# muhd-umer/ltr-lowrank-sdp

Measured on AMD Instinct MI355X. Metric: ALM iters/sec, MaxCut G67 (torus 100x100 +-1, n=m=10000), fixed default rank, higher is better.
Workload: dtype f64; 1 GPU; MaxCut torus 100x100 (G67 structure); n=10000, m=10000, rank=19, pattern_slots=30000, constraint_nnz=10000, flags=--fixedRank 19 --reoptLevel 0, phase-1 exit disabled, budget = steps, parallelism=none (1 GPU)

## Files before the change

include/lrsdp.h:

```cpp
#ifndef LRSDP_H
#define LRSDP_H
#define LRSDP_ABI_VERSION 2
#ifdef __cplusplus
extern "C" {
#endif

typedef struct lrs_ctx lrs_ctx;
typedef struct lrs_loopback lrs_loopback;

typedef struct {
    double initRho, rhoMax, rhoCellingALM, rhoCellingADMM;
    int maxALMIter, maxADMMIter;
    double timesLogRank;
    int fixedRank, initRank, rhoFreq;
    double rhoFactor, ALMRhoFactor, rankUpdateFactor, phase1Tol, phase2Tol, timeSecLimit, heuristicFactor;
    int lbfgsListLength;
    double endTauTol, endALMSubTol;
    int l2Rescaling, reoptLevel, dyrankLevel, highAccMode, oracleRankNaive;
    int disableOracle;
    double nearStallFactor;
    const int *rankSchedule;
    int rankScheduleLen;
    int verbose;
    long almInnerBudget;
    int skipADMM;
} lrs_params;

typedef struct {
    long alm_inner, alm_outer, admm_iter, cg_iter;
    double alm_pobj, alm_dobj, alm_pinf, alm_gap, alm_rho;
    double pobj, dobj, pinf, pinf_inf, gap, rho;
    double solve_time, alm_time, admm_time, read_time;
    int status;
    int retcode;
    int final_rank, oracle_rank;
    int traj1_len, traj2_len;
    double rho_max;
    double dinf, dinf_inf, dinf_2;
    int dinf_converged;
    int dinf_iters;
    long dinf_steps;
    double dinf_time;
    double obj_scale;
} lrs_result;

enum { LRS_R = 0, LRS_D = 1, LRS_G = 2, LRS_U = 3, LRS_V = 4, LRS_S0 = 5, LRS_Y0 = 6, LRS_S1 = 7, LRS_Y1 = 8 };
enum { LRS_LAMBDA = 0, LRS_CVS = 1, LRS_Q1 = 2, LRS_Q2 = 3, LRS_B = 4 };

void lrs_params_default(lrs_params *p);
const char *lrs_last_error(void);
const char *lrs_version(void);
int lrs_abi_version(void);

int lrs_ctx_create(int device, lrs_ctx **out);
void lrs_ctx_destroy(lrs_ctx *ctx);

int lrs_load_sdpa(lrs_ctx *ctx, const char *path, double *read_seconds);
int lrs_problem_info(lrs_ctx *ctx, int *m, int *ncones, int *dims, long *nslots, long *nnz_constraints);

int lrs_determine_rank(lrs_ctx *ctx, const lrs_params *p, int *ranks_out);
int lrs_set_rank(lrs_ctx *ctx, const int *ranks);
int lrs_get_rank(lrs_ctx *ctx, int *ranks);

int lrs_factor_set(lrs_ctx *ctx, int which, const double *colmajor);
int lrs_factor_get(lrs_ctx *ctx, int which, double *colmajor);
int lrs_vec_set(lrs_ctx *ctx, int which, const double *v);
int lrs_vec_get(lrs_ctx *ctx, int which, double *v);

int lrs_op_q12(lrs_ctx *ctx, double *q1, double *p1, double *q2, double *p2);
int lrs_op_constr_rr(lrs_ctx *ctx, double *cvs, double *pinf, double *pobj);
int lrs_op_grad(lrs_ctx *ctx, double rho, double *lag_norm_sq);
int lrs_op_line_search(lrs_ctx *ctx, double rho, double *tau, int *root_num);
int lrs_op_lbfgs(lrs_ctx *ctx, int node_num, double beta_new, double beta_old);
int lrs_op_admm_constr(lrs_ctx *ctx);
int lrs_op_admm_half(lrs_ctx *ctx, int cone, int side, double rho, double cg_tol, int cg_maxit, int *cg_iters,
                     double *rhs);
int lrs_op_dual_update(lrs_ctx *ctx, double rho);
int lrs_op_alm_update(lrs_ctx *ctx, double rho, double tau, double *lag_norm_sq, double *beta);
int lrs_op_adjoint(lrs_ctx *ctx, const double *y, int which, double *out, double scale, int with_C);
int lrs_op_auv(lrs_ctx *ctx, int u, int v, double *out_m, double *cobj);
int lrs_op_dimacs(lrs_ctx *ctx, int admm, double *out5);
int lrs_op_gram(lrs_ctx *ctx, int cone, int which, double *gram);
int lrs_op_dual_infeasibility(lrs_ctx *ctx, double *l1, double *lam_min);

int lrs_solve(lrs_ctx *ctx, const lrs_params *p, lrs_result *res);
int lrs_trajectory(lrs_ctx *ctx, int phase, int *curr_rank, int *oracle_rank, int cap);
int lrs_write_json(lrs_ctx *ctx, const char *path, const char *problem_id, const char *file_path,
                   const lrs_result *res, const lrs_params *p);

int lrs_alm_throughput(lrs_ctx *ctx, const lrs_params *p, long warmup, long steps, double *seconds,
                       long *done, double *sddmm_avg_ms, double *iter_avg_ms);

typedef long (*lrs_budget_hook)(void *user, long inner_done);
int lrs_set_budget_hook(lrs_ctx *ctx, lrs_budget_hook hook, void *user);
int lrs_alm_last_step(lrs_ctx *ctx, double *out4, int *newest_pair);
int lrs_sync(lrs_ctx *ctx);

int lrs_set_log_path(lrs_ctx *ctx, const char *path);

int lrs_set_kernel_path(lrs_ctx *ctx, int path);
int lrs_get_kernel_path(lrs_ctx *ctx, int *used);

int lrs_time_auut(lrs_ctx *ctx, int reps, double *avg_ms);
int lrs_auut_bytes(lrs_ctx *ctx, double *bytes);

int lrs_time_gram(lrs_ctx *ctx, int cone, int reps, double *avg_ms, double *gram_ms);

int lrs_mfma_f64_peak(lrs_ctx *ctx, double *tflops);
int lrs_mfma_f64_probe(lrs_ctx *ctx, int waves_per_simd, int chains, double *tflops, double *mhz,
                       double *cycles_per_mfma);

int lrs_time_dense(lrs_ctx *ctx, int cone, int reps, double *avg_ms);

int lrs_dense_a_info(lrs_ctx *ctx, int cone, int *n_dense, int *on_dense_path, long *stack_bytes);
int lrs_time_dense_a(lrs_ctx *ctx, int cone, int reps, double *avg_ms);
int lrs_dense_a_plan(const char *path, int cone, int *n_dense, int *on_dense_path, int *cons, int cap);

int lrs_rank1_info(lrs_ctx *ctx, int cone, int *n_rank1, int *on_factor_path, long *factor_bytes);
int lrs_rank1_plan(const char *path, int cone, int *n_rank1, int *on_factor_path, int *cons, double *sigma, int cap);
int lrs_time_rank1(lrs_ctx *ctx, int cone, int reps, double *avg_ms, double *bytes);
int lrs_load_coo_rank1(lrs_ctx *ctx, int m, int nblk, const int *dims, const double *b, long nnz, const int *con,
                       const int *blk, const int *row, const int *col, const double *val, int nterm, const int *tcon,
                       const int *tblk, const double *tsigma, const double *tvec);

int lrs_profile_stages(lrs_ctx *ctx, const lrs_params *p, long steps, double *stage_ms, long *done);

int lrs_load_coo(lrs_ctx *ctx, int m, int nblk, const int *dims, const double *b, long nnz, const int *con,
                 const int *blk, const int *row, const int *col, const double *val);

int lrs_tile_info(lrs_ctx *ctx, int *auv, int *slot);
int lrs_tile_used(lrs_ctx *ctx, int *used);

int lrs_stage_bytes(lrs_ctx *ctx, double *bytes);

int lrs_time_stages(lrs_ctx *ctx, int reps, double *stage_ms);

int lrs_debug_phase_times(lrs_ctx *ctx, unsigned long long *out, unsigned long long *blk);

int lrs_comm_unique_id(char *id_out);
int lrs_shard_rccl(lrs_ctx *ctx, int world, int rank, const char *id);
int lrs_loopback_create(int world, lrs_loopback **out);
void lrs_loopback_destroy(lrs_loopback *g);
int lrs_shard_loopback(lrs_ctx *ctx, lrs_loopback *g, int rank);
int lrs_shard_info(lrs_ctx *ctx, int *world, int *rank, int *row0, int *nown, int *nhalo);
int lrs_shard_comm_ranks(lrs_ctx *ctx, int *count);
int lrs_shard_comm_record(lrs_ctx *ctx, int on);
int lrs_xwg_fallbacks(lrs_ctx *ctx, int *count);
int lrs_shard_comm_log(lrs_ctx *ctx, long *out, long cap, long *n);
int lrs_shard_plan(const char *path, int world, int rank, long *counts, int *bounds, int *local_gid,
                   int *send_ptr, int *send_gid, int *shared_gid, int *con_gid, int *primary);

#ifdef __cplusplus
}
#endif
#endif
```

ltr-lowrank-sdp_amd/csrc/lrs_device.h:

```cpp
#pragma once
#include <hip/hip_runtime.h>

#include <cstdint>
#include <string>
#include <vector>

namespace lrs {

constexpr int kBlock = 256;
constexpr int kMaxPartialBlocks = 4096;
constexpr int kMaxPartialVals = 16;

enum CtrlIdx {
    C_ACTIVE = 0,
    C_EXIT,
    C_INNER,
    C_LOCAL,
    C_CLEAR,
    C_HEAD,
    C_GCUR,
    C_PENDING,
    C_RCVAL,
    C_LAG,
    C_PINF1,
    C_PINFINF,
    C_BETA0, C_BETA1,
    C_YY0, C_YY1,
    C_NODENUM,
    C_CG, C_CS0, C_CY0, C_CS1, C_CY1,
    C_DG,
    C_LASTTAU,
    C_DSG, C_DYG, C_DSOG, C_DYOG, C_DSOY, C_DYOY,
    C_ACT2,
    C_EXIT2,
    C_RRDONE,
    C_RCUR,
    C_NCTRL = 40
};
enum ExitReason {
    EXIT_NONE = 0,
    EXIT_CONVERGED = 1,
    EXIT_PHASE1 = 2,
    EXIT_LOCAL800 = 3,
    EXIT_TINYTAU = 4,
    EXIT_NUMERR = 5,
    EXIT_BUDGET = 6,
    EXIT_XWG = 7
};
enum ParIdx {
    P_RHO = 0, P_RCTOL, P_ENDSUB, P_ENDTAU, P_PH1TOL, P_BN1, P_BNINF, P_CNINF,
    P_HIGHACC, P_BUDGET, P_L, P_GAP, P_NPAR = 16
};
enum LsIdx { LS_TAU = 0, LS_ROOTNUM, LS_FLAG, LS_N = 4 };
constexpr int kMaxCones = 256;
constexpr int kFinN = 416;
enum TmpFinIdx {
    TF_SD = 0, TF_GATHER = 2 * kMaxCones, TF_RESID, TF_DOT, TF_DOTC, TF_SPMM = TF_DOTC + kMaxCones,
    TF_N = TF_SPMM + kMaxCones
};
constexpr int kMaxShards = 64;
constexpr int kLongRow = 32;

struct Layout {
    int G = 1, E = 1, ld = 1;
};
Layout choose_layout(int r);

struct DevCone {
    int n = 0, r = 0, ld = 0, G = 0, E = 0;
    bool lp = false;
    int *lp_slot = nullptr;
    double *lp_nrm2 = nullptr;
    int row0 = 0, nown = 0;
    long foff = 0;
    int slot_off = 0, P = 0;
    int *adj_ptr = nullptr, *adj_low = nullptr, *adj_col = nullptr, *adj_slot = nullptr;
    long adj_nnz = 0;
    bool auv_diag = false;
    int maxdeg = 0, maxlow = 0;
    std::vector<int> dra_h, drb_h;
    std::vector<int> dra_n, drb_n;
    int *dra = nullptr, *drb = nullptr;
    long gl_need = 0;
    int dense_c = 0;
    double *Cd = nullptr;
    double c_alpha = 0.0;
    int kd = 0;
    double *dA = nullptr;
    int *dA_con = nullptr;
    std::vector<int> dA_con_h;
    const double *dSd = nullptr;
    int rp = 0, rldp = 0;
    double *rV = nullptr, *r_sigma = nullptr;
    int *r_con = nullptr;
    const double *r1w = nullptr;
    double *r1T = nullptr, *r1part = nullptr;
    int *colseg = nullptr;
    int auv_items = 0;
    long auv_ebase = 0;
    int *auv_item = nullptr;
    unsigned *auv_pq = nullptr;
    int *auv_pos = nullptr;
    double *auv_val = nullptr;
    int sa_items = 0;
    int sa_n = 0;
    int *sa_item = nullptr;
    int sa_nsub = 0;
    int *sa_sub = nullptr;
    int sa_ngrp = 0;
    int *sa_grp = nullptr;
    unsigned *sa_pq = nullptr;
    int *sa_slot = nullptr;
    int sb_blocks = 0;
    int *sb_blk = nullptr, *sb_tp = nullptr, *sb_rp = nullptr, *sb_ent = nullptr;
    double *sa_S = nullptr;
    int sb_I0 = 0;
    int sx_n = 0;
    int *sx_slot = nullptr;
    int cg_ok = 0, cg_ncs = 0, cg_ncl = 0, cg_ns = 0, cg_nce = 0, cg_nsc = 0, cg_nadj = 0, cg_cconst = 0, cg_cslot = 0;
    int *cg_cadj_ptr = nullptr, *cg_cadj = nullptr, *cg_cl_con = nullptr, *cg_cl_ptr = nullptr, *cg_ce = nullptr;
    int *cg_sp = nullptr, *cg_sj = nullptr, *cg_cc_ptr = nullptr, *cg_cc = nullptr;
    double *cg_ce_w = nullptr, *cg_sa = nullptr;
    int cobj_n = 0;
    int *cobj_slot = nullptr;
};
constexpr int kScMaxN = 256;
constexpr int kMaxRankLd = 512;
constexpr int kAuvT = 128;
constexpr int kAuvC = 32;
constexpr int kAuvThreads = 512;
constexpr int kAuvNpt = 8;
constexpr int kAuvItem = kAuvThreads * kAuvNpt;
constexpr int kTileSub = 1024;
constexpr int kTileGrp = 2;
constexpr int kAuvMinN = 2048;
constexpr int kAuvMinPerTile = 768;
constexpr int kCgSplitSlabs = 8;
constexpr int kNX = 8;
constexpr int kTileMinDeg = 32;
constexpr int kDenseRow = 64;
constexpr int kSliceMinB = 28;
constexpr int kMaxDenseRows = 32;

struct ShardHooks {
    void *self = nullptr;
    int (*halo)(void *self, double *D, hipStream_t st) = nullptr;
    int (*allreduce)(void *self, double *buf, int n, hipStream_t st) = nullptr;
};

struct DevProblem {
    const ShardHooks *shard = nullptr;
    int no_lat = 0;
    int *slot_g = nullptr;
    mutable int last_path = -1;
    mutable int last_tiles = 0;
    int m = 0, K = 0;
    int lp_cone = -1;
    long NRpad = 0;
    int Ptot = 0;
    long Z = 0;
    double *b = nullptr;
    double *Cw = nullptr, *Craw = nullptr;
    int *con_ptr = nullptr, *con_slot = nullptr;
    double *con_w = nullptr;
    int *slot_ptr = nullptr, *slot_con = nullptr;
    double *slot_a = nullptr;
    int mg = 0;
    int glob_maxlen = 0;
    int *glob = nullptr;
    int *loc_ptr = nullptr, *loc_con = nullptr;
    double *loc_w = nullptr;
    int *slot_rc = nullptr;
    double *slot1 = nullptr;
    double *loc1 = nullptr;
    int *con1_pq = nullptr;
    int *long_rows = nullptr;
    std::vector<int> long_ptr_h;
    double *con1_w = nullptr;
    int nsh = 0;
    int *sh_idx = nullptr;
    double *cmask = nullptr;
    double *bprim = nullptr;
    double *g3 = nullptr;
    double *gpack = nullptr;
    double *spack = nullptr;
    std::vector<DevCone> cones;
    int ndense = 0;
    int ndensea = 0;
    bool tiles = false;
    double *gp = nullptr;
    double *cgk = nullptr;
    double dense_scale = 1.0;
    DevCone merged;
    bool has_merged = false;
    bool cone_sep = false;
};

struct DevWork {
    double *R = nullptr, *D = nullptr, *G[2] = {nullptr, nullptr};
    double *R2 = nullptr;
    double *CR = nullptr, *CD = nullptr;
    double *CGK = nullptr;
    double *dT = nullptr, *dSd = nullptr, *dpart = nullptr;
    double *rTx = nullptr, *rTz = nullptr, *rTy = nullptr, *rpart = nullptr;
    double *GP = nullptr;
    double *ls[2] = {nullptr, nullptr}, *ly[2] = {nullptr, nullptr};
    double *U = nullptr, *V = nullptr, *X = nullptr;
    double *cg_r = nullptr, *cg_p = nullptr, *cg_Q = nullptr, *cg_b = nullptr, *M2 = nullptr;
    double *uvt0 = nullptr, *uvt1 = nullptr, *uvt2 = nullptr, *S = nullptr;
    double *uvp = nullptr;
    double *lam = nullptr, *cvs = nullptr, *q1 = nullptr, *q2 = nullptr, *M1 = nullptr, *wtmp = nullptr;
    double *cvc = nullptr;
    double *lpw = nullptr;
    double *part = nullptr;
    double *partB = nullptr;
    double *partC = nullptr;
    double *ctrl = nullptr;
    double *lsres = nullptr;
    double *par = nullptr;
    double *gram = nullptr;
    double *rec = nullptr;
    double *cgc = nullptr;
    double *tot = nullptr;
    double *gl = nullptr;
    long gl_len = 0;
};


int launch_sddmm(const DevProblem &P, int cone, int mode, const double *X, const double *Y,
                 double *out0, double *out1, double *part, int pblk_off, int *nblk_used,
                 hipStream_t st);
int launch_gather(const DevProblem &P, const double *uvt, double scale, double *out,
                  const double *b_for_vio, double *vio_part, hipStream_t st, int *nblk_used);
int launch_auv_con(const DevProblem &P, int cone, int mode, const double *X, const double *Y, double scale,
                   int accumulate, double *out, const double *b_for_vio, double *vio_part, hipStream_t st,
                   const double *guard = nullptr, double *sum_upd = nullptr);
int launch_cobj(const DevProblem &P, int cone, int mode, const double *X, const double *Y, double *part,
                hipStream_t st);
// ... 103 lines not shown
```

ltr-lowrank-sdp_amd/csrc/lrs_kernels.hip:

```cpp
#include <hip/hip_runtime.h>
#include <utility>

#include <cmath>
#include <cstdio>
#include <cstring>
#include <cstdlib>
#include <algorithm>

#include "lrs_device.h"

namespace lrs {

static thread_local char g_err[512] = "";

#ifdef LRS_PHASE_TIMING
__device__ unsigned long long g_phase[4][16];
__device__ unsigned long long g_phase_tmp[4][16];
#define LRS_TS(k, p)                                                                  \
    do {                                                                              \
        if (blockIdx.x == 0 && threadIdx.x == 0) g_phase_tmp[k][p] = wall_clock64();  \
    } while (0)
#define LRS_TS_END(k, p)                                                              \
    do {                                                                              \
        if (blockIdx.x == 0 && threadIdx.x == 0) {                                    \
            g_phase_tmp[k][p] = wall_clock64();                                       \
            for (int q_ = 0; q_ <= (p); ++q_) g_phase[k][q_] = g_phase_tmp[k][q_];    \
        }                                                                             \
    } while (0)
__device__ unsigned long long g_blk[4][1024][2];
#define LRS_BLK_BEGIN() const unsigned long long t_begin_ = wall_clock64()
#define LRS_BLK_END(k)                                                                 \
    do {                                                                               \
        if (threadIdx.x == 0 && blockIdx.x < 1024) {                                   \
            g_blk[k][blockIdx.x][0] = t_begin_;                                        \
            g_blk[k][blockIdx.x][1] = wall_clock64();                                  \
        }                                                                              \
    } while (0)
#else
#define LRS_TS(k, p) do { } while (0)
#define LRS_TS_END(k, p) do { } while (0)
#define LRS_BLK_BEGIN() do { } while (0)
#define LRS_BLK_END(k) do { } while (0)
#endif
int read_phase_times(unsigned long long *out, unsigned long long *blk) {
#ifdef LRS_PHASE_TIMING
    if (hipMemcpyFromSymbol(out, HIP_SYMBOL(g_phase), sizeof(g_phase)) != hipSuccess) return -1;
    if (blk && hipMemcpyFromSymbol(blk, HIP_SYMBOL(g_blk), sizeof(g_blk)) != hipSuccess) return -1;
    return 64;
#else
    (void)out;
    (void)blk;
    return 0;
#endif
}
const char *last_device_error() { return g_err; }

#define LRS_CHECK_LAUNCH()                                                               \
    do {                                                                                 \
        hipError_t e_ = hipGetLastError();                                               \
        if (e_ != hipSuccess) {                                                          \
            snprintf(g_err, sizeof(g_err), "%s:%d %s", __FILE__, __LINE__, hipGetErrorString(e_)); \
            return (int)e_;                                                              \
        }                                                                                \
    } while (0)

Layout choose_layout(int r) {
    if (const char *e = getenv("LRS_LAYOUT")) {
        int g = 0, el = 0;
        if (sscanf(e, "%dx%d", &g, &el) == 2 && (g == 8 || g == 16 || g == 32 || g == 64) && el >= 1 && el <= 4 &&
            g * el >= r) {
            Layout f;
            f.G = g; f.E = el; f.ld = g * el;
            return f;
        }
    }
    static const int Gs[4] = {8, 16, 32, 64};
    static const int Es[4] = {2, 1, 4, 3};
    Layout best;
    best.ld = 1 << 30;
    for (int ei = 0; ei < 4; ++ei)
        for (int gi = 0; gi < 4; ++gi) {
            int ld = Gs[gi] * Es[ei];
            if (ld >= r && ld < best.ld) { best.G = Gs[gi]; best.E = Es[ei]; best.ld = ld; }
        }
    if (best.ld > 512 && r <= 512) { best.G = 64; best.E = 8; best.ld = 512; }
    return best;
}

template <int CTRL>
__device__ __forceinline__ double dpp_mov(double v) {
    const long long b = __double_as_longlong(v);
    const int lo = __builtin_amdgcn_mov_dpp((int)b, CTRL, 0xF, 0xF, false);
    const int hi = __builtin_amdgcn_mov_dpp((int)(b >> 32), CTRL, 0xF, 0xF, false);
    return __longlong_as_double(((long long)hi << 32) | (unsigned int)lo);
}

__device__ __forceinline__ double opaque(double x) {
    asm volatile("" : "+v"(x));
    return x;
}

template <int G>
__device__ __forceinline__ double group_sum(double v) {
    v += dpp_mov<0xB1>(v);
    v += dpp_mov<0x4E>(v);
    if constexpr (G >= 8) v += dpp_mov<0x141>(v);
    if constexpr (G >= 16) v += dpp_mov<0x140>(v);
    if constexpr (G >= 32) v += __shfl_xor(v, 16, 64);
    if constexpr (G >= 64) v += __shfl_xor(v, 32, 64);
    return v;
}

template <int G>
__device__ __forceinline__ double group_sum4(const double (&d)[4], int o) {
    static_assert(G == 4 || G == 16, "group of 4 or 16 lanes");
    if constexpr (G == 4) {
        const bool h1 = (o & 2) != 0, h0 = (o & 1) != 0;
        double a0 = h1 ? d[2] : d[0], a1 = h1 ? d[3] : d[1];
        a0 += dpp_mov<0x4E>(h1 ? d[0] : d[2]);
        a1 += dpp_mov<0x4E>(h1 ? d[1] : d[3]);
        return (h0 ? a1 : a0) + dpp_mov<0xB1>(h0 ? a0 : a1);
    } else {
        const bool h3 = (o & 8) != 0, h2 = (o & 4) != 0;
        double a0 = h3 ? d[2] : d[0], a1 = h3 ? d[3] : d[1];
        a0 += dpp_mov<0x140>(h3 ? d[0] : d[2]);
        a1 += dpp_mov<0x140>(h3 ? d[1] : d[3]);
        double v = (h2 ? a1 : a0) + dpp_mov<0x141>(h2 ? a0 : a1);
        v += dpp_mov<0x4E>(v);
        v += dpp_mov<0xB1>(v);
        return v;
    }
}

__device__ __forceinline__ double read_lane(double v, int l) {
    const long long b = __double_as_longlong(v);
    const int lo = __builtin_amdgcn_readlane((int)b, l);
    const int hi = __builtin_amdgcn_readlane((int)(b >> 32), l);
    return __longlong_as_double(((long long)hi << 32) | (unsigned int)lo);
}

template <int G>
__device__ __forceinline__ int bcast_i(int v, int u) {
    if constexpr (G == 64) return __builtin_amdgcn_readlane(v, u);
    else return __shfl(v, (int)(threadIdx.x & 63 & ~(G - 1)) + u, 64);
}
template <int G>
__device__ __forceinline__ double bcast_d(double v, int u) {
    if constexpr (G == 64) return read_lane(v, u);
    else return __shfl(v, (int)(threadIdx.x & 63 & ~(G - 1)) + u, 64);
}

__device__ __forceinline__ double wave_sum(double v) {
    v = group_sum<16>(v);
    return (read_lane(v, 0) + read_lane(v, 16)) + (read_lane(v, 32) + read_lane(v, 48));
}

template <int E>
__device__ __forceinline__ void ld_row(const double *__restrict__ p, double (&v)[E]) {
    if constexpr (E == 2) {
        double2 t = *reinterpret_cast<const double2 *>(p);
        v[0] = t.x; v[1] = t.y;
    } else if constexpr (E == 4) {
        double2 t0 = reinterpret_cast<const double2 *>(p)[0];
        double2 t1 = reinterpret_cast<const double2 *>(p)[1];
        v[0] = t0.x; v[1] = t0.y; v[2] = t1.x; v[3] = t1.y;
    } else {
#pragma unroll
        for (int e = 0; e < E; ++e) v[e] = p[e];
    }
}

template <int E>
__device__ __forceinline__ void st_row(double *__restrict__ p, const double (&v)[E]) {
    if constexpr (E == 2) {
        *reinterpret_cast<double2 *>(p) = make_double2(v[0], v[1]);
    } else if constexpr (E == 4) {
        reinterpret_cast<double2 *>(p)[0] = make_double2(v[0], v[1]);
        reinterpret_cast<double2 *>(p)[1] = make_double2(v[2], v[3]);
    } else {
#pragma unroll
        for (int e = 0; e < E; ++e) p[e] = v[e];
    }
}

template <int NV, int NT = kBlock>
__device__ __forceinline__ void block_reduce(double (&acc)[NV], double (&s)[NV]) {
    __shared__ double sh[NV][NT / 64];
    const int wid = threadIdx.x >> 6, lane = threadIdx.x & 63;
#pragma unroll
    for (int v = 0; v < NV; ++v) {
        double t = wave_sum(acc[v]);
        if (lane == 0) sh[v][wid] = t;
    }
    __syncthreads();
    if (threadIdx.x == 0) {
#pragma unroll
        for (int v = 0; v < NV; ++v) {
            double t = 0.0;
#pragma unroll
            for (int w = 0; w < NT / 64; ++w) t += sh[v][w];
            s[v] = t;
        }
    }
    __syncthreads();
}

template <int NV>
__device__ void partials_finalize(double (&acc)[NV], double *__restrict__ part, unsigned *ticket,
                                  double *__restrict__ fin, int *inc = nullptr) {
    double s[NV];
    block_reduce<NV>(acc, s);
    __shared__ unsigned is_last;
    if (threadIdx.x == 0) {
#pragma unroll
        for (int v = 0; v < NV; ++v) part[v * kMaxPartialBlocks + blockIdx.x] = s[v];
        asm volatile("s_waitcnt vmcnt(0)" ::: "memory");
        __builtin_amdgcn_fence(__ATOMIC_RELEASE, "agent");
        asm volatile("s_waitcnt vmcnt(0)" ::: "memory");
        unsigned t = __hip_atomic_fetch_add(ticket, 1u, __ATOMIC_RELAXED, __HIP_MEMORY_SCOPE_AGENT);
        is_last = (t == gridDim.x - 1) ? 1u : 0u;
    }
    __syncthreads();
    if (!is_last) return;
    if (threadIdx.x == 0) {
        __builtin_amdgcn_fence(__ATOMIC_ACQUIRE, "agent");
        asm volatile("s_waitcnt vmcnt(0)" ::: "memory");
    }
    __syncthreads();
    double a2[NV];
#pragma unroll
    for (int v = 0; v < NV; ++v) {
        double t = 0.0;
        for (int b = threadIdx.x; b < (int)gridDim.x; b += kBlock) t += part[v * kMaxPartialBlocks + b];
        a2[v] = t;
    }
    double s2[NV];
    block_reduce<NV>(a2, s2);
    if (threadIdx.x == 0) {
#pragma unroll
        for (int v = 0; v < NV; ++v) fin[v] = s2[v];
        if (inc) *inc = *inc + 1;
        __hip_atomic_store(ticket, 0u, __ATOMIC_RELAXED, __HIP_MEMORY_SCOPE_AGENT);
    }
}

static inline int grid_rows(long rows, int G) {
    long threads = rows * G;
    long b = (threads + kBlock - 1) / kBlock;
    if (b < 1) b = 1;
    if (b > kMaxPartialBlocks) b = kMaxPartialBlocks;
    return (int)b;
}
static inline int grid_elems(long n, int per_thread) {
    long b = (n / per_thread + kBlock - 1) / kBlock;
    if (b < 1) b = 1;
    if (b > kMaxPartialBlocks) b = kMaxPartialBlocks;
    return (int)b;
}

enum TicketId { T_SDDMM = 0, T_GATHER, T_SPMM, T_DOT, T_GRAD, T_RR, T_Q, T_NT = 16 };

// ... 816 lines not shown
    }
    if (delta < 0) {
        const double sqA = sqrt(A);
        const double T = (A * b - 1.5 * a * B) / (A * sqA);
        const double th = acos(T);
        const double cs = cos(th / 3), sn = sqrt(3.0) * sin(th / 3);
        res[0] = (-b - 2 * sqA * cs) / 3 / a;
        res[1] = (-b + sqA * (cs + sn)) / 3 / a;
        res[2] = (-b + sqA * (cs - sn)) / 3 / a;
        return 3;
    }
    return 0;
}

__device__ __forceinline__ int dev_cubic_wave(double a, double b, double c, double d, double *res) {
    const double A = b * b - 3 * a * c, B = b * c - 9 * a * d, C = c * c - 3 * b * d;
    const double delta = B * B - 4 * A * C;
    res[0] = res[1] = res[2] = 0.0;
    if (A == 0 && B == 0) { res[0] = fmax(res[0], -c / b); return 1; }
    if (delta > 0) {
        const double sq = sqrt(delta);
        const double Y1 = A * b + 1.5 * a * (-B + sq);
        const double Y2 = A * b + 1.5 * a * (-B - sq);
        const double y = (threadIdx.x & 1) ? Y2 : Y1;
        const double ay = y > 0 ? y : -y;
        double r = pow(ay, 1.0 / 3);
        r = y > 0 ? r : -r;
        const double Y13 = read_lane(r, 0), Y23 = read_lane(r, 1);
        res[0] = fmax(res[0], (-b - Y13 - Y23) / 3 / a);
        return 1;
    }
    if (delta == 0 && A != 0 && B != 0) {
        const double Kk = B / A;
        res[0] = -b / a + Kk; res[1] = -Kk / 2;
        return 2;
    }
    if (delta < 0) {
        const double sqA = sqrt(A);
        const double T = (A * b - 1.5 * a * B) / (A * sqA);
        const double th = acos(T);
        double sn, cs;
        sincos(th / 3, &sn, &cs);
        sn *= sqrt(3.0);
        res[0] = (-b - 2 * sqA * cs) / 3 / a;
        res[1] = (-b + sqA * (cs + sn)) / 3 / a;
        res[2] = (-b + sqA * (cs - sn)) / 3 / a;
        return 3;
    }
    return 0;
}

__device__ __forceinline__ double quartic(double a, double b, double c, double d, double x) {
    const double x2 = x * x;
    return a * (x2 * x2) + b * (x2 * x) + c * x2 + d * x;
}

__device__ void line_search_v(const double *__restrict__ par, double p1, double p2, const double *dots, double *ls);
__device__ void line_search(const double *__restrict__ par, int K, const double *__restrict__ fin, double *ls) {
    double p1 = 0.0, p2 = 0.0;
    for (int k = 0; k < K; ++k) { p1 += fin[FIN_SD + 2 * k]; p2 += fin[FIN_SD + 2 * k + 1]; }
    double dots[5];
    for (int q = 0; q < 5; ++q) dots[q] = fin[FIN_Q + q];
    line_search_v(par, p1, p2, dots, ls);
}
template <int NV, int NT = kBlock>
__device__ __forceinline__ void write_partials(double (&acc)[NV], double *__restrict__ part, int slot) {
    __shared__ double sh[NV][NT / 64];
    const int wid = threadIdx.x >> 6, lane = threadIdx.x & 63;
#pragma unroll
    for (int v = 0; v < NV; ++v) {
        const double t = wave_sum(acc[v]);
        if (lane == 0) sh[v][wid] = t;
    }
    __syncthreads();
    if (threadIdx.x < NV) {
        const int v = threadIdx.x;
        double t = 0.0;
#pragma unroll
        for (int w = 0; w < NT / 64; ++w) t += sh[v][w];
        part[v * kMaxPartialBlocks + slot] = t;
    }
}

template <int NV>
__device__ __forceinline__ void write_partials_nw(double (&acc)[NV], double *__restrict__ part, int slot, int nw) {
    __shared__ double sh[NV][8];
    const int wid = threadIdx.x >> 6, lane = threadIdx.x & 63;
#pragma unroll
    for (int v = 0; v < NV; ++v) {
        const double t = wave_sum(acc[v]);
        if (lane == 0) sh[v][wid] = t;
    }
    __syncthreads();
    if (threadIdx.x < NV) {
        const int v = threadIdx.x;
        double t = 0.0;
#pragma unroll
        for (int w = 0; w < 8; ++w)
            if (w < nw) t += sh[v][w];
        part[v * kMaxPartialBlocks + slot] = t;
    }
}

template <int NV, int NT = kBlock>
__device__ __forceinline__ void write_partials_range(double (&acc)[NV], double *__restrict__ part, int slot, int v0,
                                                     int v1) {
    double s[NV];
    block_reduce<NV, NT>(acc, s);
    if (threadIdx.x == 0) {
#pragma unroll
        for (int v = 0; v < NV; ++v)
            if (v >= v0 && v < v1) part[v * kMaxPartialBlocks + slot] = s[v];
    }
}

template <int NV, int NT = kBlock>
__device__ __forceinline__ void reduce_partials(const double *__restrict__ part, int nblk, double *out,
                                                int pstr = kMaxPartialBlocks) {
    double a[NV];
#pragma unroll
    for (int v = 0; v < NV; ++v) a[v] = 0.0;
    for (int b = threadIdx.x; b < nblk; b += NT) {
#pragma unroll
        for (int v = 0; v < NV; ++v) a[v] += part[v * pstr + b];
    }
    double s[NV];
    block_reduce<NV, NT>(a, s);
    if (threadIdx.x == 0) {
#pragma unroll
        for (int v = 0; v < NV; ++v) out[v] = s[v];
    }
    __syncthreads();
}

template <bool WAVE, typename PB>
__device__ __forceinline__ void line_search_t(const PB &par, double p1, double p2, const double *dots, double *ls) {
    p1 *= 2.0;
    const double rho = par[P_RHO];
    const double a = rho * dots[0] / 2;
    const double b = rho * dots[1];
    const double c = p2 - rho * dots[2] + rho * dots[3] / 2;
    const double d = p1 - rho * dots[4];
    double roots[3];
    const int rn = WAVE ? dev_cubic_wave(4 * a, 3 * b, 2 * c, d, roots) : dev_cubic(4 * a, 3 * b, 2 * c, d, roots);
    double tau = 0.0;
    const double f0 = 0.0, f1 = quartic(a, b, c, d, 1.0);
    double fr1 = 1e30, fr2 = 1e30, fr3 = 1e30;
    if (rn >= 1 && roots[0] > 1e-20 && roots[0] <= 1.0) fr1 = quartic(a, b, c, d, roots[0]);
    if (rn >= 2 && roots[1] > 1e-20 && roots[1] <= 1.0) fr2 = quartic(a, b, c, d, roots[1]);
    if (rn == 3 && roots[2] > 1e-20 && roots[2] <= 1.0) fr3 = quartic(a, b, c, d, roots[2]);
    const double mn = fmin(fmin(fmin(fmin(f0, f1), fr1), fr2), fr3);
    if (fabs(mn - f0) < 1e-10) tau = 0.0;
    if (fabs(mn - f1) < 1e-10) tau = 1.0;
    if (fabs(mn - fr1) < 1e-10) tau = roots[0];
    if (fabs(mn - fr2) < 1e-10) tau = roots[1];
    if (fabs(mn - fr3) < 1e-10) tau = roots[2];
    if (!WAVE || (threadIdx.x & 63) == 0) {
        ls[LS_TAU] = tau;
        ls[LS_ROOTNUM] = rn;
        ls[LS_FLAG] = rn == 0 ? 1.0 : (fabs(tau) < par[P_ENDTAU] ? 2.0 : 0.0);
    }
}
__device__ void line_search_v(const double *__restrict__ par, double p1, double p2, const double *dots, double *ls) {
    line_search_t<false>(par, p1, p2, dots, ls);
}

template <typename CB, typename PB>
__device__ __forceinline__ void ctrl_step(CB &&c, const PB &par, double lsflag, double lstau, int fold,
                                          const double *d, bool ph1) {
    const int L = (int)par[P_L];
    const double cninf = par[P_CNINF], rctol = par[P_RCTOL], endsub = par[P_ENDSUB], budget = par[P_BUDGET];
    c[C_ACTIVE] = c[C_ACT2];
    c[C_EXIT] = c[C_EXIT2];
    c[C_RRDONE] = 0.0;
    if (c[C_ACTIVE] != 0.0 && c[C_PENDING] == 1.0) {
        if (lsflag == 1.0) {
            c[C_ACTIVE] = 0.0; c[C_EXIT] = EXIT_NUMERR;
            c[C_PENDING] = 0.0;
        } else if (lsflag == 2.0) {
            c[C_INNER] += 1; c[C_LOCAL] += 1; c[C_CLEAR] += 1;
            c[C_ACTIVE] = 0.0; c[C_EXIT] = EXIT_TINYTAU;
            c[C_PENDING] = 0.0;
        } else if (fold) {
            const int h = (int)c[C_HEAD];
// ... 998 lines not shown
            }
            st_row<E>(CRb + foff + oi, cr);
        }
        double sv2[E], yv[E];
#pragma unroll
        for (int e = 0; e < E; ++e) g[e] *= 2.0;
#pragma unroll
        for (int e = 0; e < E; ++e) { sv2[e] = tau * w.di[e]; yv[e] = g[e] - go[e]; }
        st_row<E>(Gnew + oi, g);
        st_row<E>(sh + oi, sv2);
        st_row<E>(yh + oi, yv);
#pragma unroll
        for (int e = 0; e < E; ++e) {
            acc[0] += g[e] * g[e];
            acc[1] += yv[e] * sv2[e];
            acc[2] += yv[e] * yv[e];
            acc[3] += sv2[e] * g[e];
            acc[4] += yv[e] * g[e];
        }
        if (two) {
#pragma unroll
            for (int e = 0; e < E; ++e) {
                acc[5] += sov[e] * g[e];
                acc[6] += yov[e] * g[e];
                acc[7] += sov[e] * yv[e];
                acc[8] += yov[e] * yv[e];
            }
        }
    }
    LRS_TS(2, 3);
    write_partials<10, kRowBlock>(acc, partC, pblk_off + blockIdx.x);
    LRS_TS_END(2, 4);
    LRS_BLK_END(2);
}

__device__ __forceinline__ int lat_row_block(int b, int nrb) {
#ifndef LRS_NO_LAT_XCD
    if (b >= nrb || nrb < 16) return b;
    const int x = b & 7, q8 = nrb >> 3, rem = nrb & 7;
    const int start = x * q8 + min(x, rem);
    return start + (b >> 3);
#else
    (void)nrb;
    return b;
#endif
}
constexpr int kLatNT = 512;
constexpr int kLatRowWaves = kLatNT / 64 - 1;
constexpr int kLatRows = kLatRowWaves * 64;
constexpr int kLatMaxPartials = 256;
constexpr int kSliceA = 2;
constexpr int kSliceB = 4;

constexpr int kLatQ = kLatMaxPartials / 64;
template <int NV>
__device__ __forceinline__ void load_partials(const double *__restrict__ part, int nblk, double (&x)[kLatQ][NV]) {
    const int lane = threadIdx.x & 63;
#pragma unroll
    for (int q = 0; q < kLatQ; ++q) {
        const int bc = min(lane + 64 * q, nblk - 1);
#pragma unroll
        for (int v = 0; v < NV; ++v) x[q][v] = part[v * kMaxPartialBlocks + bc];
    }
}
template <int NV>
__device__ __forceinline__ void sum_partials(const double (&x)[kLatQ][NV], int nblk, double (&out)[NV]) {
    const int lane = threadIdx.x & 63;
#pragma unroll
    for (int v = 0; v < NV; ++v) {
        double a = 0.0;
#pragma unroll
        for (int q = 0; q < kLatQ; ++q) a += (lane + 64 * q < nblk) ? x[q][v] : 0.0;
        out[v] = wave_sum(a);
    }
}
template <int NV>
__device__ __forceinline__ void wave_reduce_partials(const double *__restrict__ part, int nblk, double (&out)[NV]) {
    double x[kLatQ][NV];
    load_partials<NV>(part, nblk, x);
    __builtin_amdgcn_sched_barrier(0);
    sum_partials<NV>(x, nblk, out);
}

template <int G, int E, int NO>
__global__ void __launch_bounds__(kLatNT) k_lat_a(
    int n, int ld, long foff, const int *__restrict__ adj_ptr, const int *__restrict__ adj_low,
    const int *__restrict__ adj_col, const int *__restrict__ adj_slot, const double *__restrict__ Cw,
    const double *__restrict__ Rb0, const double *__restrict__ Rb1, double *__restrict__ Dall,
    const double *__restrict__ G0, const double *__restrict__ G1, const double *__restrict__ s0a,
    const double *__restrict__ y0a, const double *__restrict__ s1a, const double *__restrict__ y1a,
    double *__restrict__ uRD, double *__restrict__ uDD, const int *__restrict__ loc_ptr,
    const int *__restrict__ loc_con, const double *__restrict__ loc_w, const double2 *__restrict__ loc1,
    const double *__restrict__ b, double *__restrict__ cvs, const double *__restrict__ lam,
    double *__restrict__ rec, int do_glob, int mg, const int *__restrict__ glob, int m, int K,
    const int *__restrict__ con_ptr, const int *__restrict__ con_slot, const double *__restrict__ con_w,
    const double *__restrict__ uRR, const double *__restrict__ par, const double *__restrict__ ctrl_prev,
    double *__restrict__ ctrl_cur, const double *__restrict__ ls_prev, const double *__restrict__ partC, int nblkC,
    double *__restrict__ partA, int pblk_off, int gwide, int nrb, int lrw, int nda, const int *__restrict__ dra) {
    __shared__ double c[C_NCTRL];
    __shared__ double pl[P_NPAR];
    LRS_TS(0, 0);
    LRS_BLK_BEGIN();
    const int nwv = lrw + 1, rpb = lrw * 64 / G;
    const bool ctrl_wave = __builtin_amdgcn_readfirstlane((int)(threadIdx.x >> 6)) == nwv - 1;
    const int lane = threadIdx.x & (G - 1);
    const bool slice = (int)blockIdx.x >= nrb;
    int i = lat_row_block((int)blockIdx.x, nrb) * rpb + (int)threadIdx.x / G, sq = 0;
    if (slice) {
        const int per = rpb * kSliceA;
        int q = (int)blockIdx.x - nrb, L = 0;
        for (; L < nda - 1; ++L) {
            const int r = dra[L], ns = (adj_low[r] - adj_ptr[r] + per - 1) / per;
            if (q < ns) break;
            q -= ns;
        }
        i = dra[L];
        sq = q * per + ((int)threadIdx.x / G) * kSliceA;
    }
    const bool valid = !ctrl_wave && i < n;
    const int ic = valid ? i : 0;
    double px[kLatQ][10], ccv = 0.0, pvv = 0.0;
    int kb = 0, ke = 0;
    if (ctrl_wave) {
        load_partials<10>(partC, nblkC, px);
        const int l64 = threadIdx.x & 63;
        ccv = ctrl_prev[min(l64, C_NCTRL - 1)];
        pvv = par[min(l64, P_NPAR - 1)];
    } else {
        kb = adj_ptr[ic];
        ke = adj_low[ic];
    }
    __builtin_amdgcn_sched_barrier(0);
    const double lsflag = ls_prev[LS_FLAG];
    const int fold = (ctrl_prev[C_ACT2] != 0.0 && ctrl_prev[C_PENDING] == 1.0 && lsflag == 0.0) ? 1 : 0;
#ifdef LRS_PHASE_TIMING
    if (blockIdx.x == 0 && threadIdx.x == 0 && kb != -12345) g_phase_tmp[0][10] = wall_clock64();
    if (blockIdx.x == 0 && threadIdx.x == 0 && fold != 12345) g_phase_tmp[0][9] = wall_clock64();
    if (blockIdx.x == 0 && ctrl_wave && (threadIdx.x & 63) == 0 && ccv != 12345.678) g_phase_tmp[0][11] = wall_clock64();
#endif
    const bool r1 = (ctrl_prev[C_RCUR] != 0.0) != (fold != 0);
    const bool g1 = (ctrl_prev[C_GCUR] != 0.0) != (fold != 0);
    const double *__restrict__ R = (r1 ? Rb1 : Rb0) + foff;
    const double *__restrict__ Gc = (g1 ? G1 : G0) + foff;
    const double *__restrict__ s0 = s0a + foff, *__restrict__ y0 = y0a + foff;
    const double *__restrict__ s1 = s1a + foff, *__restrict__ y1 = y1a + foff;
    double *__restrict__ D = Dall + foff;
    const long oi = (long)ic * ld + lane * E;
    DirRow<E> own;
    double xi[E];
    int no = 0;
    bool dg = false;
    int jj[NO], ss[NO];
    double cw[NO], bq[NO], cq[NO], lq[NO];
    double2 l1[NO];
    DirRow<E> nbr[NO];
    double xj[NO][E];
    int sd = 0;
    double cwd = 0.0, bd = 0.0, cd = 0.0, lmd = 0.0;
    double2 l1d = make_double2(0.0, -1.0);
    if (ctrl_wave) {
        const int l64 = threadIdx.x & 63;
        if (l64 < C_NCTRL) c[l64] = ccv;
        if (l64 < P_NPAR) pl[l64] = pvv;
        double s[10];
        if (fold) {
            sum_partials<10>(px, nblkC, s);
        } else {
#pragma unroll
            for (int v = 0; v < 10; ++v) s[v] = 0.0;
        }
#ifdef LRS_PHASE_TIMING
        if (blockIdx.x == 0 && l64 == 0 && s[9] != 12345.678 && ccv != 12345.678) g_phase_tmp[0][8] = wall_clock64();
#endif
        {
            double cr[C_NCTRL], pr[P_NPAR];
#pragma unroll
            for (int q = 0; q < C_NCTRL; ++q) cr[q] = c[q];
#pragma unroll
            for (int q = 0; q < P_NPAR; ++q) pr[q] = pl[q];
            ctrl_step(cr, pr, lsflag, ls_prev[LS_TAU], fold, s, mg == 0);
            if (l64 == 0) {
#pragma unroll
                for (int q = 0; q < C_NCTRL; ++q) c[q] = cr[q];
            }
        }
#ifdef LRS_PHASE_TIMING
        if (blockIdx.x == 0 && l64 == 0) g_phase_tmp[0][7] = wall_clock64();
#endif
    } else {
        ld_row<E>(Gc + oi, own.g);
        ld_row<E>(s0 + oi, own.a0); ld_row<E>(y0 + oi, own.b0);
        ld_row<E>(s1 + oi, own.a1); ld_row<E>(y1 + oi, own.b1);
        ld_row<E>(R + oi, xi);
        int eb = kb, nl = valid ? ke - kb : 0;
        if (slice) { eb = kb + sq; nl = valid ? max(0, min(kSliceA, ke - eb)) : 0; }
        else if (nl > kDenseRow) nl = 0;
        const int kd = nl > 0 ? eb + nl - 1 : 0;
        const int jd = adj_col[kd];
        sd = adj_slot[kd];
#pragma unroll
        for (int u = 0; u < NO; ++u) {
            const int k = nl > 0 ? eb + min(u, nl - 1) : 0;
            jj[u] = adj_col[k];
            ss[u] = adj_slot[k];
        }
        kb = eb;
        dg = !slice && nl > 0 && jd == i;
        no = nl - (dg ? 1 : 0);
        cwd = Cw[sd];
        l1d = loc1[sd];
#pragma unroll
        for (int u = 0; u < NO; ++u) {
            cw[u] = Cw[ss[u]];
            l1[u] = loc1[ss[u]];
            const long oj = (long)(u < no ? jj[u] : ic) * ld + lane * E;
            ld_row<E>(R + oj, xj[u]);
            ld_row<E>(Gc + oj, nbr[u].g);
            ld_row<E>(s0 + oj, nbr[u].a0); ld_row<E>(y0 + oj, nbr[u].b0);
            ld_row<E>(s1 + oj, nbr[u].a1); ld_row<E>(y1 + oj, nbr[u].b1);
        }
        const int ispare = min(ic, m - 1);
#pragma unroll
        for (int u = 0; u < NO; ++u) {
            const int ci = (int)l1[u].y >= 0 ? (int)l1[u].y : ispare;
            bq[u] = b[ci];
            cq[u] = cvs[ci];
            lq[u] = lam[ci];
        }
        {
            const int ci = (int)l1d.y >= 0 ? (int)l1d.y : ispare;
            bd = b[ci];
            cd = cvs[ci];
            lmd = lam[ci];
        }
#ifdef LRS_PHASE_TIMING
        if (blockIdx.x == 0 && threadIdx.x == 0 && xi[0] != 12345.678) g_phase_tmp[0][1] = wall_clock64();
        if (blockIdx.x == 0 && threadIdx.x == 0 && bq[0] != 12345.678 && xj[0][0] != 12345.678 && bd != 12345.678)
            g_phase_tmp[0][2] = wall_clock64();
#endif
    }
    __syncthreads();
    LRS_TS(0, 3);
    if (pblk_off == 0 && blockIdx.x == 0 && threadIdx.x < C_NCTRL) ctrl_cur[threadIdx.x] = c[threadIdx.x];
    const bool active = c[C_ACTIVE] != 0.0;
    if (!active && !(fold && mg > 0)) return;
    double acc[8] = {0, 0, 0, 0, 0, 0, 0, 0};
    if (fold && do_glob) {
        if (gwide) {
            const int lane64 = threadIdx.x & 63;
            const int nw = gridDim.x * nwv;
            for (int g = blockIdx.x * nwv + (threadIdx.x >> 6); g < mg; g += nw) {
                const int ig = glob[g];
                double tot = 0.0;
                for (int k = 0; k < K; ++k) {
                    const long row = (long)k * m + ig;
                    double v = 0.0;
                    for (int e = con_ptr[row] + lane64; e < con_ptr[row + 1]; e += 64) v += con_w[e] * uRR[con_slot[e]];
                    tot += wave_sum(v);
                }
                if (lane64 == 0) {
                    cvs[ig] = tot;
                    const double dd = b[ig] - tot;
                    acc[7] += dd * dd;
                }
            }
        } else {
            for (int g = blockIdx.x * nwv * 64 + threadIdx.x; g < mg; g += gridDim.x * nwv * 64) {
                const int ig = glob[g];
                double tot = 0.0;
                for (int k = 0; k < K; ++k) {
                    const long row = (long)k * m + ig;
                    double v = 0.0;
                    for (int e = con_ptr[row]; e < con_ptr[row + 1]; ++e) v += con_w[e] * uRR[con_slot[e]];
                    tot += v;
                }
                cvs[ig] = tot;
                const double dd = b[ig] - tot;
                acc[7] += dd * dd;
            }
        }
    }
    if (active && valid) {
        DirCoef kc;
        kc.cg = c[C_CG]; kc.cs0 = c[C_CS0]; kc.cy0 = c[C_CY0]; kc.cs1 = c[C_CS1]; kc.cy1 = c[C_CY1];
        kc.u0 = (kc.cs0 != 0.0 || kc.cy0 != 0.0);
        kc.u1 = (kc.cs1 != 0.0 || kc.cy1 != 0.0);
        const double rho = par[P_RHO], rhoInv = 1.0 / rho;
        double yi[E];
        own.eval(kc, yi);
        if (!slice) st_row<E>(D + oi, yi);
        auto entry = [&](int j, int sl, const double (&xjv)[E], const double (&yj)[E], double cwv, double2 l1v,
                         double bv, double cv, double lv) {
            double d0 = 0.0, d1 = 0.0;
            if (j != i) {
#pragma unroll
                for (int e = 0; e < E; ++e) d0 += xi[e] * yj[e] + xjv[e] * yi[e];
                d0 *= 0.5;
            } else {
#pragma unroll
                for (int e = 0; e < E; ++e) d0 += xi[e] * yi[e];
            }
#pragma unroll
            for (int e = 0; e < E; ++e) d1 += yi[e] * yj[e];
            d0 = group_sum<G>(d0);
            d1 = group_sum<G>(d1);
            if (lane != 0) return;
            uRD[sl] = d0;
            uDD[sl] = d1;
            acc[0] += cwv * d0;
            acc[1] += cwv * d1;
            const int c1 = (int)l1v.y;
            const int e0 = c1 == -2 ? loc_ptr[sl] : 0, e1 = c1 == -2 ? loc_ptr[sl + 1] : (c1 >= 0 ? 1 : 0);
            for (int e = e0; e < e1; ++e) {
                const int ci = c1 >= 0 ? c1 : loc_con[e];
                const double w = c1 >= 0 ? l1v.x : loc_w[e];
                const double bi = c1 >= 0 ? bv : b[ci], cvi = c1 >= 0 ? cv : cvs[ci], li = c1 >= 0 ? lv : lam[ci];
                const double q1 = 2.0 * (w * d0), q2 = w * d1;
                const double q0 = (bi - cvi) + rhoInv * li;
                acc[2] += q2 * q2; acc[3] += q1 * q2; acc[4] += q0 * q2; acc[5] += q1 * q1;
                acc[6] += q0 * q1;
                double2 *r = reinterpret_cast<double2 *>(rec + 4L * ci);
                r[0] = make_double2(cvi, q1);
                r[1] = make_double2(q2, (-li) + (-rho) * bi);
            }
        };
#pragma unroll
        for (int u = 0; u < NO; ++u) {
            if (u < no) {
                double yj[E];
                nbr[u].eval(kc, yj);
                entry(jj[u], ss[u], xj[u], yj, cw[u], l1[u], bq[u], cq[u], lq[u]);
            }
        }
        for (int k = kb + NO; k < kb + no; ++k) {
            const int j = adj_col[k], sl = adj_slot[k];
            const long oj = (long)j * ld + lane * E;
            double xjv[E], yj[E];
            ld_row<E>(R + oj, xjv);
            DirRow<E> dj;
            dj.load(kc, Gc, s0, y0, s1, y1, oj);
            dj.eval(kc, yj);
            const double2 l1v = loc1[sl];
            const int ci = (int)l1v.y;
            double bv = 0.0, cv = 0.0, lv = 0.0;
            if (ci >= 0) { bv = b[ci]; cv = cvs[ci]; lv = lam[ci]; }
            entry(j, sl, xjv, yj, Cw[sl], l1v, bv, cv, lv);
        }
        if (dg) entry(i, sd, xi, yi, cwd, l1d, bd, cd, lmd);
    }
    LRS_TS(0, 5);
    write_partials_nw<8>(acc, partA, pblk_off + blockIdx.x, nwv);
    LRS_TS_END(0, 6);
#ifdef LRS_PHASE_TIMING
    if (blockIdx.x == 0 && threadIdx.x == 0)
        for (int q_ = 7; q_ < 12; ++q_) g_phase[0][q_] = g_phase_tmp[0][q_];
#endif
    LRS_BLK_END(0);
}

template <int G, int E, int NO>
__global__ void __launch_bounds__(kLatNT) k_lat_b(
    int n, int ld, long foff, const int *__restrict__ adj_ptr, const int *__restrict__ adj_low,
    const int *__restrict__ adj_col, const int *__restrict__ adj_slot, double *Rb0, double *Rb1,
    const double *__restrict__ Dall, double *G0, double *G1, double *s0, double *y0, double *s1, double *y1,
    double *__restrict__ uRR, const double *__restrict__ Craw, const int *__restrict__ slot_ptr,
    const int *__restrict__ slot_con, const double *__restrict__ slot_a, const double2 *__restrict__ slot1,
    const double *__restrict__ rec, const int *__restrict__ loc_ptr, const int *__restrict__ loc_con,
    const double *__restrict__ loc_w, const double2 *__restrict__ loc1, const double *__restrict__ b,
    double *__restrict__ cvs, const double *__restrict__ par, const double *__restrict__ ctrl,
    const double *__restrict__ partA, int nblkA, const double *__restrict__ partB, int nblkB,
    double *__restrict__ ls_cur, int L, double *__restrict__ partC, int pblk_off, int m, double *hmirror,
    double seq, int nrb, int lrw, int ndb, const int *__restrict__ drb, double *__restrict__ gl, double *CRb,
    const double *__restrict__ CDb) {
    __shared__ double red[12];
    __shared__ double ls[LS_N];
    __shared__ double pl[P_NPAR];
    __shared__ double gsh[kLatRows * E];
    LRS_TS(2, 0);
    LRS_BLK_BEGIN();
    mirror_ctrl(ctrl, hmirror, seq);
    const int nwv = lrw + 1, rpb = lrw * 64 / G;
    const bool ctrl_wave = __builtin_amdgcn_readfirstlane((int)(threadIdx.x >> 6)) == nwv - 1;
    const int lane = threadIdx.x & (G - 1);
    const bool slice = (int)blockIdx.x >= nrb;
    int i = lat_row_block((int)blockIdx.x, nrb) * rpb + (int)threadIdx.x / G, sq = 0;
    if (slice) {
        const int per = rpb * kSliceB;
        int q = (int)blockIdx.x - nrb, Ld = 0;
        for (; Ld < ndb - 1; ++Ld) {
            const int r = drb[Ld], ns = (adj_ptr[r + 1] - adj_ptr[r] + per - 1) / per;
            if (q < ns) break;
            q -= ns;
        }
        i = drb[Ld];
        sq = q * per + ((int)threadIdx.x / G) * kSliceB;
    }
    const bool valid = !ctrl_wave && i < n;
    const int ic = valid ? i : 0;
    double pa[kLatQ][7], pb[kLatQ][5], pvv = 0.0;
    int kb = 0, kl = 0, ke = 0;
    if (ctrl_wave) {
        load_partials<7>(partA, nblkA, pa);
        if (nblkB > 0) load_partials<5>(partB, nblkB, pb);
        pvv = par[min((int)(threadIdx.x & 63), P_NPAR - 1)];
    } else {
        kb = adj_ptr[ic];
        kl = adj_low[ic];
        ke = adj_ptr[ic + 1];
    }
    __builtin_amdgcn_sched_barrier(0);
    if (ctrl[C_ACT2] == 0.0) return;
    const int gcur = (int)ctrl[C_GCUR], h = (int)ctrl[C_HEAD];
    const bool r1 = ctrl[C_RCUR] != 0.0;
    const double *__restrict__ R = (r1 ? Rb1 : Rb0) + foff;
    double *__restrict__ Rn = (r1 ? Rb0 : Rb1) + foff;
    const double *__restrict__ D = Dall + foff;
    double *__restrict__ Gold = (gcur == 0 ? G0 : G1) + foff;
    double *__restrict__ Gnew = (gcur == 0 ? G1 : G0) + foff;
    double *__restrict__ sh = (h == 0 ? s0 : s1) + foff;
    double *__restrict__ yh = (h == 0 ? y0 : y1) + foff;
    const double *__restrict__ so = (h == 0 ? s1 : s0) + foff;
    const double *__restrict__ yo = (h == 0 ? y1 : y0) + foff;
    const bool two = (L == 2);
    const long oi = (long)ic * ld + lane * E;
    int no = 0;
    bool dg = false, dense = false;
    double ri[E], di[E], go[E], sov[E], yov[E];
    int ss[NO];
    bool lw[NO];
    double rjp[NO][E], djp[NO][E];
    double sv[NO], bq[NO];
    double2 s1v[NO], l1v[NO], ra[NO], rb[NO];
    int sd = 0;
    double svd = 0.0, bqd = 0.0;
    double2 s1d = make_double2(0.0, -1.0), l1d = s1d, rad = make_double2(0.0, 0.0), rbd = rad;
    const double *__restrict__ RA = R;
    if (ctrl_wave) {
        double sA[7];
        sum_partials<7>(pa, nblkA, sA);
        if (nblkB > 0) {
            double sB[5];
            sum_partials<5>(pb, nblkB, sB);
#pragma unroll
            for (int q = 0; q < 5; ++q) sA[2 + q] += sB[q];
        }
        if ((threadIdx.x & 63) == 0) {
#pragma unroll
            for (int v = 0; v < 7; ++v) red[v] = sA[v];
        }
        __builtin_amdgcn_wave_barrier();
#ifdef LRS_PHASE_TIMING
        if (blockIdx.x == 0 && (threadIdx.x & 63) == 0 && sA[6] != 12345.678) g_phase_tmp[2][8] = wall_clock64();
#endif
        if ((threadIdx.x & 63) < P_NPAR) pl[threadIdx.x & 63] = pvv;
        __builtin_amdgcn_wave_barrier();
        line_search_t<true>(pl, red[0], red[1], red + 2, ls);
#ifdef LRS_PHASE_TIMING
        if (blockIdx.x == 0 && (threadIdx.x & 63) == 0) g_phase_tmp[2][7] = wall_clock64();
#endif
    } else {
        ld_row<E>(R + oi, ri);
        ld_row<E>(D + oi, di);
        ld_row<E>(Gold + oi, go);
        if (two) { ld_row<E>(so + oi, sov); ld_row<E>(yo + oi, yov); }
        int eb = kb, nt = valid ? ke - kb : 0;
        if (slice) { eb = kb + sq; nt = valid ? max(0, min(kSliceB, ke - eb)) : 0; }
        else if (nt > kDenseRow) { nt = 0; dense = true; }
        const int kd = (!slice && nt > 0 && kl > kb) ? kl - 1 : 0;
        const int jd = adj_col[kd];
        sd = adj_slot[kd];
        int ja[NO + 1], sa[NO + 1];
#pragma unroll
        for (int u = 0; u <= NO; ++u) {
            const int k = nt > 0 ? eb + min(u, nt - 1) : 0;
            ja[u] = adj_col[k];
            sa[u] = adj_slot[k];
        }
        dg = !slice && nt > 0 && kl > kb && jd == i;
        no = nt - (dg ? 1 : 0);
        const int pd = dg ? kl - 1 - kb : NO + 1;
#pragma unroll
        for (int u = 0; u < NO; ++u) {
            const bool past = u >= pd;
            const int j = past ? ja[u + 1] : ja[u];
            ss[u] = past ? sa[u + 1] : sa[u];
            lw[u] = eb + u + (past ? 1 : 0) < kl;
            const long oj = (long)(u < no ? j : ic) * ld + lane * E;
            ld_row<E>(RA + oj, rjp[u]);
            ld_row<E>(D + oj, djp[u]);
            sv[u] = Craw[ss[u]];
            s1v[u] = slot1[ss[u]];
            l1v[u] = loc1[ss[u]];
        }
        svd = Craw[sd];
        s1d = slot1[sd];
        l1d = loc1[sd];
        const int ispare = min(ic, m - 1);
#pragma unroll
        for (int u = 0; u < NO; ++u) {
            const int c1 = (int)s1v[u].y >= 0 ? (int)s1v[u].y : ispare;
            const int cl = (int)l1v[u].y >= 0 ? (int)l1v[u].y : ispare;
            const double2 *r = reinterpret_cast<const double2 *>(rec + 4L * c1);
            ra[u] = r[0];
            rb[u] = r[1];
            bq[u] = b[cl];
        }
        {
            const int c1 = (int)s1d.y >= 0 ? (int)s1d.y : ispare;
            const int cl = (int)l1d.y >= 0 ? (int)l1d.y : ispare;
            const double2 *r = reinterpret_cast<const double2 *>(rec + 4L * c1);
            rad = r[0];
            rbd = r[1];
            bqd = b[cl];
        }
#ifdef LRS_PHASE_TIMING
        if (blockIdx.x == 0 && threadIdx.x == 0 && ri[0] != 12345.678 && sv[0] != 12345.678)
            g_phase_tmp[2][5] = wall_clock64();
        if (blockIdx.x == 0 && threadIdx.x == 0 && bq[0] != 12345.678 && ra[0].x != 12345.678 && rjp[0][0] != 12345.678)
            g_phase_tmp[2][6] = wall_clock64();
#endif
    }
    __syncthreads();
    LRS_TS(2, 2);
    if (pblk_off == 0 && blockIdx.x == 0 && threadIdx.x < LS_N) ls_cur[threadIdx.x] = ls[threadIdx.x];
    if (ls[LS_FLAG] != 0.0) return;
    const double tau = ls[LS_TAU], tau2 = tau * tau, rho = par[P_RHO];
    double acc[10] = {0, 0, 0, 0, 0, 0, 0, 0, 0, 0};
    double g[E];
#pragma unroll
    for (int e = 0; e < E; ++e) g[e] = 0.0;
    if (valid) {
#pragma unroll
        for (int e = 0; e < E; ++e) ri[e] += tau * di[e];
        if (!slice) st_row<E>(Rn + oi, ri);
        auto entry = [&](int sl, bool lower, const double (&rj)[E], double svv, double2 s1u, double2 ra_, double2 rb_,
                         double2 l1u, double bv) {
            const int c1 = (int)s1u.y;
            const int e0 = c1 == -2 ? slot_ptr[sl] : 0;
            const int e1 = c1 == -2 ? slot_ptr[sl + 1] : (c1 >= 0 ? 1 : 0);
            for (int e = e0; e < e1; ++e) {
                double2 x = ra_, y = rb_;
                if (c1 < 0) {
                    const double2 *r = reinterpret_cast<const double2 *>(rec + 4L * slot_con[e]);
                    x = r[0];
                    y = r[1];
                }
                double cv = x.x + tau * x.y;
                cv = cv + tau2 * y.x;
                const double M1 = y.y + rho * cv;
                svv += M1 * (c1 >= 0 ? s1u.x : slot_a[e]);
            }
#pragma unroll
            for (int e = 0; e < E; ++e) g[e] += svv * rj[e];
            if (!lower) return;
            double d = 0.0;
#pragma unroll
            for (int e = 0; e < E; ++e) d += ri[e] * rj[e];
            d = group_sum<G>(d);
            if (lane != 0) return;
            uRR[sl] = d;
            const int cl = (int)l1u.y;
            const int f0 = cl == -2 ? loc_ptr[sl] : 0;
            const int f1 = cl == -2 ? loc_ptr[sl + 1] : (cl >= 0 ? 1 : 0);
            for (int e = f0; e < f1; ++e) {
                const int ci = cl >= 0 ? cl : loc_con[e];
                const double tot = (cl >= 0 ? l1u.x : loc_w[e]) * d;
                cvs[ci] = tot;
                const double dd = (cl >= 0 ? bv : b[ci]) - tot;
                acc[9] += dd * dd;
            }
        };
#pragma unroll
        for (int u = 0; u < NO; ++u) {
            if (u < no) {
                double rj[E];
#pragma unroll
                for (int e = 0; e < E; ++e) rj[e] = rjp[u][e] + tau * djp[u][e];
                entry(ss[u], lw[u], rj, sv[u], s1v[u], ra[u], rb[u], l1v[u], bq[u]);
            }
        }
        if (!slice && no > NO) {
            int cnt = 0;
            for (int k = kb; k < ke; ++k) {
                if (dg && k == kl - 1) continue;
                if (cnt++ < NO) continue;
                const int j = adj_col[k], sl = adj_slot[k];
                const long oj = (long)j * ld + lane * E;
                double rj[E], dj[E];
                ld_row<E>(R + oj, rj);
                ld_row<E>(D + oj, dj);
#pragma unroll
                for (int e = 0; e < E; ++e) rj[e] += tau * dj[e];
                const double2 s1u = slot1[sl];
                const int c1 = (int)s1u.y;
                double2 x = make_double2(0.0, 0.0), y = x;
                if (c1 >= 0) {
                    const double2 *r = reinterpret_cast<const double2 *>(rec + 4L * c1);
                    x = r[0];
                    y = r[1];
                }
                const bool lower = k < kl;
                const double2 l1u = lower ? loc1[sl] : make_double2(0.0, -1.0);
                const int cl = (int)l1u.y;
                entry(sl, lower, rj, Craw[sl], s1u, x, y, l1u, cl >= 0 ? b[cl] : 0.0);
            }
        }
        if (dg) entry(sd, true, ri, svd, s1d, rad, rbd, l1d, bqd);
        if (!slice && !dense) {
            double sv2[E], yv[E];
            if (CRb) {
                double cr[E], cd[E];
                ld_row<E>(CRb + foff + oi, cr);
                ld_row<E>(CDb + foff + oi, cd);
#pragma unroll
                for (int e = 0; e < E; ++e) {
                    cr[e] += tau * cd[e];
                    g[e] += cr[e];
                }
                st_row<E>(CRb + foff + oi, cr);
            }
#pragma unroll
            for (int e = 0; e < E; ++e) g[e] *= 2.0;
#pragma unroll
            for (int e = 0; e < E; ++e) { sv2[e] = tau * di[e]; yv[e] = g[e] - go[e]; }
            st_row<E>(Gnew + oi, g);
            st_row<E>(sh + oi, sv2);
            st_row<E>(yh + oi, yv);
#pragma unroll
            for (int e = 0; e < E; ++e) {
                acc[0] += g[e] * g[e];
                acc[1] += yv[e] * sv2[e];
                acc[2] += yv[e] * yv[e];
                acc[3] += sv2[e] * g[e];
                acc[4] += yv[e] * g[e];
            }
            if (two) {
#pragma unroll
                for (int e = 0; e < E; ++e) {
                    acc[5] += sov[e] * g[e];
                    acc[6] += yov[e] * g[e];
                    acc[7] += sov[e] * yv[e];
                    acc[8] += yov[e] * yv[e];
                }
            }
        }
    }
    if (slice) {
        if (!ctrl_wave) {
#pragma unroll
            for (int e = 0; e < E; ++e) gsh[threadIdx.x * E + e] = g[e];
        }
        __syncthreads();
        if ((int)threadIdx.x < G * E) {
            const int ln = threadIdx.x / E, e = threadIdx.x % E;
            double t = 0.0;
            for (int q = 0; q < rpb; ++q) t += gsh[(q * G + ln) * E + e];
            gl[(long)((int)blockIdx.x - nrb) * ld + threadIdx.x] = t;
        }
    }
    LRS_TS(2, 3);
    write_partials_nw<10>(acc, partC, pblk_off + blockIdx.x, nwv);
    LRS_TS_END(2, 4);
#ifdef LRS_PHASE_TIMING
    if (blockIdx.x == 0 && threadIdx.x == 0)
        for (int q_ = 5; q_ < 12; ++q_) g_phase[2][q_] = g_phase_tmp[2][q_];
#endif
    LRS_BLK_END(2);
}

__global__ void __launch_bounds__(kRowBlock) k_lat_f(
    int ld, int w, long foff, const int *__restrict__ adj_ptr, const int *__restrict__ drb, int per,
    const double *__restrict__ gl, const double *__restrict__ Dall, double *G0, double *G1, double *s0, double *y0,
    double *s1, double *y1, const double *__restrict__ ctrl, const double *__restrict__ ls_cur, int L,
    double *__restrict__ partC, int pblk_off, double *CRb, const double *__restrict__ CDb) {
    if (ctrl[C_ACT2] == 0.0 || ls_cur[LS_FLAG] != 0.0) return;
    const int gcur = (int)ctrl[C_GCUR], h = (int)ctrl[C_HEAD];
    const double *__restrict__ D = Dall + foff;
    const double *__restrict__ Gold = (gcur == 0 ? G0 : G1) + foff;
    double *__restrict__ Gnew = (gcur == 0 ? G1 : G0) + foff;
    double *__restrict__ sh = (h == 0 ? s0 : s1) + foff;
    double *__restrict__ yh = (h == 0 ? y0 : y1) + foff;
    const double *__restrict__ so = (h == 0 ? s1 : s0) + foff;
    const double *__restrict__ yo = (h == 0 ? y1 : y0) + foff;
    const double tau = ls_cur[LS_TAU];
    int sl0 = 0;
    for (int q = 0; q < (int)blockIdx.x; ++q) {
        const int r = drb[q];
        sl0 += (adj_ptr[r + 1] - adj_ptr[r] + per - 1) / per;
    }
    const int i = drb[blockIdx.x], ns = (adj_ptr[i + 1] - adj_ptr[i] + per - 1) / per;
    double acc[10] = {0, 0, 0, 0, 0, 0, 0, 0, 0, 0};
    const int t = threadIdx.x;
    if (t < w) {
        const long oi = (long)i * ld + t;
        double g = 0.0;
        for (int q = 0; q < ns; ++q) g += gl[(long)(sl0 + q) * ld + t];
        if (CRb) {
            const double cr = CRb[foff + oi] + tau * CDb[foff + oi];
            CRb[foff + oi] = cr;
            g += cr;
        }
        g *= 2.0;
        const double sv2 = tau * D[oi], yv = g - Gold[oi];
        Gnew[oi] = g;
        sh[oi] = sv2;
        yh[oi] = yv;
        acc[0] = g * g;
        acc[1] = yv * sv2;
        acc[2] = yv * yv;
        acc[3] = sv2 * g;
        acc[4] = yv * g;
        if (L == 2) {
            const double sov = so[oi], yov = yo[oi];
            acc[5] = sov * g;
            acc[6] = yov * g;
            acc[7] = sov * yv;
            acc[8] = yov * yv;
        }
    }
    write_partials<10, kRowBlock>(acc, partC, pblk_off + blockIdx.x);
}


__device__ __forceinline__ void tile_rows(bool tl, int &grp, int &ngrp, int &xg, int G) {
    if (tl) {
        xg = blockIdx.x & (kNX - 1);
        const int bq = blockIdx.x / kNX, nbq = ((int)gridDim.x - xg + kNX - 1) / kNX;
        grp = (bq * kRowBlock + (int)threadIdx.x) / G;
        ngrp = nbq * kRowBlock / G;
    } else {
        xg = 0;
        grp = (blockIdx.x * kRowBlock + (int)threadIdx.x) / G;
        ngrp = gridDim.x * kRowBlock / G;
    }
}

template <int G, int E, int U, bool TL>
__global__ void __launch_bounds__(kRowBlock) k_wide_a(
    int n, int ld, long foff, const int *__restrict__ adj_ptr, const int *__restrict__ adj_low,
    const int *__restrict__ adj_col, const int *__restrict__ adj_slot, const double *__restrict__ Cw,
    const double *__restrict__ Rb0, const double *__restrict__ Rb1, const double *__restrict__ Dall,
    double *__restrict__ uRD, double *__restrict__ uDD, const int *__restrict__ loc_ptr,
    const int *__restrict__ loc_con, const double *__restrict__ loc_w, const double2 *__restrict__ loc1,
    const double *__restrict__ b, const double *__restrict__ cvs, const double *__restrict__ lam,
// ... 2330 lines not shown
    }
    return v != 0;
}
template <int GG, int EE, int UU>
static int res_b(bool fused = false) {
    static int c = 0;
    if constexpr (UU == 1) {
        static int c0 = 0, c1 = 0;
        const int r = resident_blocks(k_it_b<GG, EE, 1, 2>, &c);
        if (!fused) return r;
        const int r0 = std::min(r, resident_blocks(k_it_b<GG, EE, LRS_BW_UB, 0>, &c0));
        return bw_b_on() ? std::min(r0, resident_blocks(k_bw_b<GG, EE, kBwNo>, &c1)) : r0;
    }
    return resident_blocks(k_it_b<GG, EE, UU, (UU == 1 ? 2 : 0)>, &c);
}

constexpr int kWideU = 8;
struct StagePlan {
    int grid = 1;
    bool small = true;
    int T = 1;
    bool wide = false;
    bool afused = false;
};
static int team_size(const DevCone &c, double deg, int U) {
    const long cap_threads = 256L * 2048;
    int T = 1;
    while (T * 2 <= kRowBlock / c.G && (double)(T * 2 * U) <= deg && (long)c.nown * T * 2 * c.G <= cap_threads)
        T *= 2;
    return T;
}
static int forced_regime() {
    static int v = -1;
    if (v < 0) {
        const char *e = getenv("LRS_FORCE_REGIME");
        v = !e ? 0 : (strcmp(e, "small") == 0 ? 1 : (strcmp(e, "large") == 0 ? 2 : 0));
    }
    return v;
}
#ifndef LRS_BW_U
#define LRS_BW_U 1
#endif
constexpr int kBwU = LRS_BW_U;
static StagePlan plan_stage(long rows_threads, int res_small, int res_large, int K, int T, int force) {
    StagePlan p;
    p.T = T;
    const long need = std::max(1L, (rows_threads * T + kRowBlock - 1) / kRowBlock);
    const int cap = std::max(1, kMaxPartialBlocks / std::max(1, K));
    const int fr = force >= 2 ? 2 : forced_regime();
    if (fr == 2) { p.grid = (int)std::max(1L, std::min<long>(std::min<long>(need, res_large), cap)); p.small = false; return p; }
    if (fr == 1) { p.grid = (int)std::max(1L, std::min<long>(need, cap)); p.small = true; return p; }
    if (need <= res_small) { p.grid = (int)std::min<long>(need, cap); p.small = true; }
    else { p.grid = (int)std::min<long>(std::min<long>(need, res_large), cap); p.small = false; }
    p.grid = std::max(1, p.grid);
    return p;
}
static int plan_a(const DevCone &c, int K, StagePlan &p, int force, bool sharded) {
    const double deg = c.nown > 0 ? (double)c.P / c.nown : 0.0;
    const int T = team_size(c, deg, 2);
    const bool wide_rows = (deg / T >= 32.0 || force == 3) && c.E <= 2;
    const bool fused = a_fused_rows(c, T, wide_rows, sharded);
    LRS_LAYOUT_SWITCH(c.G, c.E, {
        p = plan_stage((long)c.nown * c.G, res_a<GG, EE, 2>(), res_a<GG, EE, 1>(fused), K, T, force);
    });
    p.wide = !p.small && wide_rows;
    p.afused = !p.small && fused;
    return 0;
}
static int plan_b(const DevCone &c, int K, StagePlan &p, int force, bool fused) {
    const double deg = c.nown > 0 ? (double)c.adj_nnz / c.nown : 0.0;
    const int T = team_size(c, deg, 4);
    const bool wide_rows = (deg / T >= 64.0 || force == 3) && c.E <= 2;
    LRS_LAYOUT_SWITCH(c.G, c.E, {
        p = plan_stage((long)c.nown * c.G, res_b<GG, EE, 4>(), res_b<GG, EE, 1>(fused && !wide_rows), K, T, force);
    });
    p.wide = !p.small && (deg / T >= 64.0 || force == 3) && c.E <= 2;
    return 0;
}

constexpr int kLatNoA = 2, kLatNoB = 4;
template <int GG, int EE>
static int res_la() {
    static int c = 0;
    return resident_blocks(k_lat_a<GG, EE, kLatNoA>, &c, kLatNT);
}
template <int GG, int EE>
static int res_lb() {
    static int c = 0;
    return resident_blocks(k_lat_b<GG, EE, kLatNoB>, &c, kLatNT);
}
static bool lat_disabled() {
    static int v = -1;
    if (v < 0) {
        const char *e = getenv("LRS_NO_LAT");
        v = (e && atoi(e) != 0) ? 1 : 0;
    }
    return v != 0;
}
struct LatPlan {
    int nrb = 0, sa = 0, sb = 0, nf = 0, nt = kLatNT;
};
static int lat_slices(const std::vector<int> &cnt, int per) {
    int s = 0;
    for (int x : cnt) s += (x + per - 1) / per;
    return s;
}
static int lat_resident(const DevCone &c, int &ra, int &rb) {
    LRS_LAYOUT_SWITCH(c.G, c.E, { ra = (res_la<GG, EE>)(); rb = (res_lb<GG, EE>)(); });
    return 0;
}
static LatPlan lat_plan(const DevCone &c, const StagePlan &pa, const StagePlan &pb, int w = kLatRowWaves) {
    LatPlan lp;
    if (lat_disabled() || forced_regime() == 2 || c.maxdeg <= 0 || !pa.small || !pb.small || pa.T != 1 || pb.T != 1)
        return lp;
    if ((int)c.dra_h.size() > kMaxDenseRows || (int)c.drb_h.size() > kMaxDenseRows) return lp;
    const int rows = 64 * w;
    const long need = std::max(1L, ((long)c.nown * c.G + rows - 1) / rows);
    const int sa = lat_slices(c.dra_n, (rows / c.G) * kSliceA);
    const int sb = lat_slices(c.drb_n, (rows / c.G) * kSliceB);
    int ra = 0, rb = 0;
    if (lat_resident(c, ra, rb)) return lp;
    if (need + sa > ra || need + sb > rb || need + sa > kLatMaxPartials) return lp;
    if (need + sb + (long)c.drb_h.size() > kLatMaxPartials) return lp;
    lp.nrb = (int)need;
    lp.sa = sa;
    lp.sb = sb;
    lp.nf = (int)c.drb_h.size();
    lp.nt = 64 * (w + 1);
    return lp;
}
static int lat_forced_waves() {
    static int forced = -1;
    if (forced < 0) {
        const char *e = getenv("LRS_LAT_ROWWAVES");
        forced = e ? std::max(0, std::min(kLatRowWaves, atoi(e))) : 0;
    }
    return forced;
}

static int multi_path(const DevProblem &P) { return P.no_lat == 4 ? 0 : P.no_lat; }

bool alm_stage_a_split(const DevProblem &P) {
    for (int k = 0; k < P.K; ++k) {
        StagePlan pa;
        if (plan_a(P.cones[k], P.K, pa, multi_path(P), P.shard != nullptr)) return false;
        if (!pa.small && !pa.afused) return true;
    }
    return false;
}

static bool b_fused_on() {
    static int v = -1;
    if (v < 0) {
        const char *e = getenv("LRS_B_FUSED");
        v = (e && e[0] == '0') ? 0 : 1;
    }
    return v != 0;
}
bool alm_stage_b_split(const DevProblem &P) {
    for (int k = 0; k < P.K; ++k) {
        StagePlan pb;
        if (plan_b(P.cones[k], P.K, pb, multi_path(P), !P.shard && b_fused_on())) return false;
        if (!pb.small && (pb.wide || P.shard || !b_fused_on())) return true;
    }
    return false;
}

int enqueue_alm_iteration(const AlmIterArgs &a, int parity, hipStream_t st) {
    return enqueue_alm_stages(a, parity, 7, st);
}

template <int NV, int NT = kRowBlock>
__global__ void __launch_bounds__(NT) k_fold_partials(const double *__restrict__ part, int nblk,
                                                      double *__restrict__ out) {
    __shared__ double red[NV];
    reduce_partials<NV, NT>(part, nblk, red);
    if (threadIdx.x < NV) out[threadIdx.x] = red[threadIdx.x];
}
int sync_shared(const DevProblem &P, double *v, hipStream_t st) {
    if (!P.shard || P.nsh == 0) return 0;
    const ShardHooks *sh = P.shard;
    hipLaunchKernelGGL(k_fill, dim3(grid_elems(P.nsh, 4)), dim3(kBlock), 0, st, (long)P.nsh, 0.0, P.spack);
    hipLaunchKernelGGL(k_pack_shared, dim3(grid_elems(P.m, 1)), dim3(kBlock), 0, st, P.m, P.sh_idx, v, P.spack, 0);
    LRS_CHECK_LAUNCH();
    if (sh->allreduce(sh->self, P.spack, P.nsh, st)) return -1;
    hipLaunchKernelGGL(k_pack_shared, dim3(grid_elems(P.m, 1)), dim3(kBlock), 0, st, P.m, P.sh_idx, v, P.spack, 1);
    LRS_CHECK_LAUNCH();
    return 0;
}
struct CtrlPut { double v[P_NPAR + C_NCTRL]; };
__global__ void k_put_ctrl(CtrlPut c, double *__restrict__ par, double *__restrict__ ctl) {
    const int t = threadIdx.x;
    if (t < P_NPAR) par[t] = c.v[t];
    if (t < C_NCTRL) ctl[t] = c.v[P_NPAR + t];
}
int launch_put_ctrl(const double *par, const double *ctl, double *dpar, double *dctl, hipStream_t st) {
    CtrlPut c;
    for (int q = 0; q < P_NPAR; ++q) c.v[q] = par[q];
    for (int q = 0; q < C_NCTRL; ++q) c.v[P_NPAR + q] = ctl[q];
    hipLaunchKernelGGL(k_put_ctrl, dim3(1), dim3(64), 0, st, c, dpar, dctl);
    LRS_CHECK_LAUNCH();
    return 0;
}

int launch_fold1(const double *part, int nblk, double *out, hipStream_t st) {
    hipLaunchKernelGGL((k_fold_partials<1, kBlock>), dim3(1), dim3(kBlock), 0, st, part, nblk, out);
    LRS_CHECK_LAUNCH();
    return 0;
}

int enqueue_alm_stages(const AlmIterArgs &a, int parity, int mask, hipStream_t st) {
    const DevProblem &P = *a.P;
    DevWork &W = *a.W;
// ... 5 lines not shown
    const ShardHooks *sh = P.shard;
    if (sh && !W.tot) {
        snprintf(g_err, sizeof(g_err), "sharded iteration: no totals buffer");
        return -1;
    }
    bool merge = P.K > 1 && P.has_merged && !sh;
    for (int k = 1; k < P.K && merge; ++k)
        merge = P.cones[k].G == P.cones[0].G && P.cones[k].E == P.cones[0].E && P.cones[k].ld == P.cones[0].ld;
    DevCone mc;
    if (merge) {
        mc = P.merged;
        mc.G = P.cones[0].G; mc.E = P.cones[0].E; mc.ld = P.cones[0].ld; mc.r = P.cones[0].r;
        mc.foff = 0;
    }
    const int KL = merge ? 1 : P.K;
    auto cone_of = [&](int k) -> const DevCone & { return merge ? mc : P.cones[k]; };
    StagePlan pa[kMaxCones], pb[kMaxCones];
    int nblkA = 0, nblkB = 0;
    bool split = sh != nullptr;
    for (int k = 0; k < KL; ++k) {
        if (plan_a(cone_of(k), KL, pa[k], multi_path(P), sh != nullptr) ||
            plan_b(cone_of(k), KL, pb[k], multi_path(P), !sh && b_fused_on()))
            return -1;
        nblkA += pa[k].grid;
        nblkB += pb[k].grid;
        if (!pa[k].small && !pa[k].afused) split = true;
    }
    bool tla[kMaxCones], tlb[kMaxCones];
    auto bfused = [&](const StagePlan &pl, bool tiled) { return b_fused_on() && !sh && !pl.small && !pl.wide && !tiled; };
    int offBF = nblkB;
    for (int k = 0; k < KL; ++k) {
        const bool can = P.tiles && !merge && !sh && W.GP && cone_of(k).colseg && cone_of(k).nown >= kNX;
        tla[k] = can && pa[k].wide && pa[k].grid >= kNX;
        tlb[k] = can && pb[k].wide && pb[k].grid >= kNX;
        if (tlb[k]) nblkB += pb[k].grid;
    }
    bool tbt[kMaxCones];
    for (int k = 0; k < KL; ++k) {
        tbt[k] = !merge && !tlb[k] && pb[k].wide && W.GP && cone_of(k).sb_blocks > 0 && cone_of(k).sa_items > 0;
        if (tbt[k]) nblkB += pb[k].grid;
    }
    if (nblkB > kMaxPartialBlocks) {
        snprintf(g_err, sizeof(g_err), "stage B: %d partial blocks past %d", nblkB, kMaxPartialBlocks);
        return -1;
    }
    const bool use_uvp = !sh && !merge && KL == 1 && W.uvp && split && pa[0].wide && !tla[0] &&
                         cone_of(0).sa_items > 0;
    double2 *uvp = use_uvp ? reinterpret_cast<double2 *>(W.uvp) : nullptr;
    const int gwide = P.glob_maxlen >= 32 ? 1 : 0;
    const int gg = gwide ? std::min((std::max(1, P.mg) + kBlock / 64 - 1) / (kBlock / 64), kMaxPartialBlocks)
                         : std::min(grid_elems(std::max(1, P.mg), 1), kMaxPartialBlocks);
    LatPlan lg[kMaxCones];
    const int ngd = P.ndense ? dense_cd_blocks(P) : 0;
    bool lat = !sh && !split && !multi_path(P);
    int nla = 0, nlb = 0, nlf = 0;
    for (int k = 0; k < KL && lat; ++k) {
        lg[k] = lat_plan(cone_of(k), pa[k], pb[k]);
        if (lg[k].nrb <= 0) lat = false;
    }
    if (lat) {
        const int cap = std::min(kLatMaxPartials, num_cus());
        const int wf = lat_forced_waves();
        for (int w = wf > 0 ? wf : 1; w <= kLatRowWaves; ++w) {
            nla = nlb = nlf = 0;
            bool fits = true;
            for (int k = 0; k < KL; ++k) {
                lg[k] = lat_plan(cone_of(k), pa[k], pb[k], w);
                if (lg[k].nrb <= 0) fits = false;
                nla += lg[k].nrb + lg[k].sa;
                nlb += lg[k].nrb + lg[k].sb;
                nlf += lg[k].nf;
            }
            if (wf > 0 || w == kLatRowWaves) {
                lat = fits;
                break;
            }
            if (fits && nla + ngd <= cap && nlb + nlf <= cap && (P.mg == 0 || gg <= cap)) break;
        }
    }
    if (lat && (nla + ngd > kLatMaxPartials || nlb + nlf > kLatMaxPartials || (P.mg > 0 && gg > kLatMaxPartials)))
        lat = false;
    P.last_path = lat ? 0 : 1;
    P.last_tiles = 0;
    for (int k = 0; k < KL; ++k)
        if (tbt[k] || (pa[k].wide && !merge && !tla[k] && cone_of(k).sa_items > 0)) P.last_tiles = 1;
    if (lat) {
        nblkA = nla;
        nblkB = nlb + nlf;
        for (int k = 0; k < KL; ++k) {
            pa[k].grid = lg[k].nrb + lg[k].sa;
            pb[k].grid = lg[k].nrb + lg[k].sb;
        }
    }
    const int offCD = nblkA;
    if (ngd) {
        nblkA += ngd;
        if (nblkA > kMaxPartialBlocks) {
            snprintf(g_err, sizeof(g_err), "dense objective: %d partial blocks past %d", nblkA, kMaxPartialBlocks);
            return -1;
        }
    }
    const bool totals = sh != nullptr;
    double *totA = totals ? W.tot : nullptr, *totC = totals ? W.tot + 16 : nullptr;
    const double *inC = totals ? totC : W.partC;
    const int nC = totals ? 1 : nblkB, pstr = totals ? 1 : kMaxPartialBlocks;
    const double *inA = totals ? totA : W.part;
    const int nA = totals ? 1 : nblkA;
    auto mark = [&](int q) -> int {
        if (a.ev && hipEventRecord(a.ev[q], st) != hipSuccess) {
            snprintf(g_err, sizeof(g_err), "hipEventRecord failed");
            return -1;
        }
        return 0;
    };
#define LRS_WIDE_A(TL_)                                                                                        \
    hipLaunchKernelGGL((k_wide_a<GG, EE, kWideU, TL_>), dim3(grid), dim3(kRowBlock), 0, st, c.nown, c.ld, c.foff,   \
                       c.adj_ptr, c.adj_low, c.adj_col, c.adj_slot, P.Cw, W.R, W.R2, W.D, W.uvt0, W.uvt1, P.loc_ptr,  \
                       P.loc_con, P.loc_w, reinterpret_cast<const double2 *>(P.loc1), P.b, W.cvs, W.lam, W.rec,      \
                       W.par, ctrl_cur, W.part, off, c.row0, P.m, c.colseg)
#define LRS_WIDE_B(TL_)                                                                                        \
    hipLaunchKernelGGL((k_wide_b<GG, EE, kWideU, TL_>), dim3(grid), dim3(kRowBlock), 0, st, c.nown, c.ld, c.foff,   \
                       c.adj_ptr, c.adj_low, c.adj_col, c.adj_slot, W.R, W.R2, W.D, W.G[0], W.G[1], W.ls[0], W.ly[0], \
                       W.ls[1], W.ly[1], W.uvt2, P.Craw, P.slot_ptr, P.slot_con, P.slot_a,                          \
                       reinterpret_cast<const double2 *>(P.slot1), W.rec, P.loc_ptr, P.loc_con, P.loc_w,             \
                       reinterpret_cast<const double2 *>(P.loc1), P.b, W.cvs, W.par, ctrl_cur, ls_cur, L, W.partC,   \
                       off, c.row0, P.m, P.ndense ? W.CR : nullptr, W.CD, c.colseg, W.GP, P.NRpad)
    if (mark(0)) return -1;
    int off = 0;
    for (int k = 0; k < KL && (mask & 1); ++k) {
        const DevCone &c = cone_of(k);
        const int grid = pa[k].grid;
#define LRS_LAUNCH_A(UU, MM)                                                                               \
    hipLaunchKernelGGL((k_it_a<GG, EE, UU, MM>), dim3(grid), dim3(kRowBlock), 0, st, c.nown, c.ld, c.foff,     \
                       c.adj_ptr, c.adj_low, c.adj_col, c.adj_slot, P.Cw, W.R, W.R2, W.D, W.G[0], W.G[1], W.ls[0], \
                       W.ly[0], W.ls[1], W.ly[1], W.uvt0, W.uvt1, P.loc_ptr, P.loc_con, P.loc_w,                \
                       reinterpret_cast<const double2 *>(P.loc1), P.b, W.cvs,                                     \
                       W.lam, W.rec, (k == 0 && !sh) ? 1 : 0, P.mg, P.glob, P.m, P.K, P.con_ptr, P.con_slot,       \
                       P.con_w,                                                                                   \
                       W.uvt2, W.par, ctrl_prev, ctrl_cur, ls_prev, inC, nC, W.part, off, pa[k].T, gwide, c.row0, \
                       pstr)
        if (lat) {
            LRS_LAYOUT_SWITCH(c.G, c.E, {
                hipLaunchKernelGGL((k_lat_a<GG, EE, kLatNoA>), dim3(grid), dim3(lg[k].nt), 0, st, c.nown,
                                   c.ld, c.foff, c.adj_ptr, c.adj_low, c.adj_col, c.adj_slot, P.Cw, W.R, W.R2, W.D,
                                   W.G[0], W.G[1], W.ls[0], W.ly[0], W.ls[1], W.ly[1], W.uvt0, W.uvt1, P.loc_ptr,
                                   P.loc_con, P.loc_w, reinterpret_cast<const double2 *>(P.loc1), P.b, W.cvs, W.lam,
                                   W.rec, k == 0 ? 1 : 0, P.mg, P.glob, P.m, P.K, P.con_ptr, P.con_slot, P.con_w,
                                   W.uvt2, W.par, ctrl_prev, ctrl_cur, ls_prev, inC, nC, W.part, off, gwide,
                                   lg[k].nrb, lg[k].nt / 64 - 1, (int)c.dra_h.size(), c.dra);
            });
        } else {
            LRS_LAYOUT_SWITCH(c.G, c.E, {
                if (split) LRS_LAUNCH_A(1, 1);
                else if (pa[k].small) LRS_LAUNCH_A(2, 0);
                else LRS_LAUNCH_A(1, 0);
            });
        }
        LRS_CHECK_LAUNCH();
        off += grid;
    }
    if (sh && (mask & 1) && sh->halo(sh->self, W.D, st)) return -1;
    off = 0;
    for (int k = 0; k < KL && (mask & 1) && split; ++k) {
        const DevCone &c = cone_of(k);
        const int grid = pa[k].grid;
        if (pa[k].wide && !merge && !tla[k] && c.sa_items > 0) {
            static int rca = 0;
            const int nwork = std::min(grid, resident_blocks(k_tile_a, &rca, 1024));
            hipLaunchKernelGGL(k_tile_a, dim3(grid), dim3(1024), 0, st, c.n, c.r, c.ld, c.foff, c.sa_ngrp, c.sa_grp,
                               nwork, reinterpret_cast<const int4 *>(c.sa_sub), c.sa_pq, c.sa_slot, P.Cw, W.R, W.R2,
                               W.D, W.uvt0, W.uvt1, P.loc_ptr, P.loc_con, P.loc_w,
                               reinterpret_cast<const double2 *>(P.loc1), P.b, W.cvs, W.lam, W.rec, W.par, ctrl_cur,
                               W.part, off, uvp);
        } else if (pa[k].wide) {
            LRS_LAYOUT_SWITCH(c.G, c.E, {
                if (tla[k]) LRS_WIDE_A(true);
                else LRS_WIDE_A(false);
            });
        } else {
            LRS_LAYOUT_SWITCH(c.G, c.E, { LRS_LAUNCH_A(kBwU, 2); });
        }
        LRS_CHECK_LAUNCH();
        off += grid;
    }
#undef LRS_LAUNCH_A
    if (ngd && (mask & 1) && launch_dense_cd(P, W, ctrl_cur, offCD, st)) return -1;
    if (totals && (mask & 1)) {
        hipLaunchKernelGGL(k_fold_partials<8>, dim3(1), dim3(kRowBlock), 0, st, W.part, nblkA, totA);
        LRS_CHECK_LAUNCH();
        if (sh && sh->allreduce(sh->self, totA, 8, st)) return -1;
    }
    if (mark(1)) return -1;
    double *totB = totals ? W.tot + 8 : nullptr;
    if (sh && P.mg > 0 && (mask & 2)) {
        const int g1 = gwide ? gg : std::min(grid_elems(P.mg, 1), kMaxPartialBlocks);
        if (P.nsh > 0) {
            hipLaunchKernelGGL(k_fill, dim3(grid_elems(3L * P.nsh, 4)), dim3(kBlock), 0, st, 3L * P.nsh, 0.0, P.gpack);
            LRS_CHECK_LAUNCH();
        }
        hipLaunchKernelGGL(k_g_part, dim3(g1), dim3(kBlock), 0, st, P.mg, P.glob, P.m, P.K, P.con_ptr, P.con_slot, P.con_w,
                           W.uvt2, W.uvt0, W.uvt1, P.sh_idx, P.g3, P.gpack, gwide, ctrl_cur);
        LRS_CHECK_LAUNCH();
        if (P.nsh > 0 && sh->allreduce(sh->self, P.gpack, 3 * P.nsh, st)) return -1;
        const int g2 = std::min(grid_elems(P.mg, 1), kMaxPartialBlocks);
        hipLaunchKernelGGL(k_it_g_sh, dim3(g2), dim3(kBlock), 0, st, P.mg, P.glob, P.m, P.sh_idx, P.g3, P.gpack, P.cmask,
                           P.b, W.cvs, W.lam, W.par, ctrl_cur, W.rec, W.partB);
        LRS_CHECK_LAUNCH();
        hipLaunchKernelGGL(k_fold_partials<6>, dim3(1), dim3(kRowBlock), 0, st, W.partB, g2, totB);
        LRS_CHECK_LAUNCH();
        if (sh->allreduce(sh->self, totB, 6, st)) return -1;
        hipLaunchKernelGGL(k_g_ph1, dim3(1), dim3(64), 0, st, W.par, ctrl_cur, totC, totB);
        LRS_CHECK_LAUNCH();
    } else if (P.mg > 0 && (mask & 2)) {
        hipLaunchKernelGGL(k_it_g, dim3(gg), dim3(kBlock), 0, st, P.mg, P.glob, P.m, P.K, P.con_ptr, P.con_slot,
                           P.con_w, W.uvt0, W.uvt1, P.b, W.cvs, W.lam, W.par, ctrl_cur, W.partC, nblkB, W.part,
                           nblkA, W.rec, W.partB, gwide, uvp);
        LRS_CHECK_LAUNCH();
    }
    if (mark(2)) return -1;
    off = 0;
    long glo = 0;
    for (int k = 0; k < KL && (mask & 4); ++k) {
        const DevCone &c = cone_of(k);
        const int grid = pb[k].grid;
#define LRS_LAUNCH_B(UU, MM)                                                                               \
    hipLaunchKernelGGL((k_it_b<GG, EE, UU, MM>), dim3(grid), dim3(kRowBlock), 0, st, c.nown, c.ld, c.foff, c.adj_ptr, \
                       c.adj_low, c.adj_col, c.adj_slot, W.R, W.R2, W.D, W.G[0], W.G[1], W.ls[0], W.ly[0],        \
                       W.ls[1], W.ly[1], W.uvt2, P.Craw, P.slot_ptr, P.slot_con, P.slot_a,                        \
                       reinterpret_cast<const double2 *>(P.slot1), W.rec, P.loc_ptr, P.loc_con, P.loc_w,           \
                       reinterpret_cast<const double2 *>(P.loc1), P.b, W.cvs, W.par, ctrl_cur, inA, nA,            \
                       sh ? totB : W.partB, P.mg > 0 ? (sh ? 1 : gg) : 0, ls_cur, L, W.partC, off, pb[k].T, c.row0, \
                       c.n, pstr,                                                                                 \
                       (MM) != 2 && k == 0 ? a.hmirror : nullptr, a.seq, P.ndense ? W.CR : nullptr, W.CD)
        const bool small = pb[k].small;
        if (lat) {
            LRS_LAYOUT_SWITCH(c.G, c.E, {
                hipLaunchKernelGGL((k_lat_b<GG, EE, kLatNoB>), dim3(grid), dim3(lg[k].nt), 0, st, c.nown,
                                   c.ld, c.foff, c.adj_ptr, c.adj_low, c.adj_col, c.adj_slot, W.R, W.R2, W.D, W.G[0],
                                   W.G[1], W.ls[0], W.ly[0], W.ls[1], W.ly[1], W.uvt2, P.Craw, P.slot_ptr, P.slot_con,
                                   P.slot_a, reinterpret_cast<const double2 *>(P.slot1), W.rec, P.loc_ptr, P.loc_con,
                                   P.loc_w, reinterpret_cast<const double2 *>(P.loc1), P.b, W.cvs, W.par, ctrl_cur,
                                   inA, nA, W.partB, P.mg > 0 ? gg : 0, ls_cur, L, W.partC, off, P.m,
                                   k == 0 ? a.hmirror : nullptr, a.seq, lg[k].nrb, lg[k].nt / 64 - 1, (int)c.drb_h.size(), c.drb,
                                   W.gl + glo, P.ndense ? W.CR : nullptr, W.CD);
            });
            glo += (long)lg[k].sb * c.ld;
        } else {
            LRS_LAYOUT_SWITCH(c.G, c.E, {
                if (small) LRS_LAUNCH_B(4, 0);
                else if (bfused(pb[k], tbt[k]) && pb[k].T == 1 && bw_b_on())
                    hipLaunchKernelGGL((k_bw_b<GG, EE, kBwNo>), dim3(grid), dim3(kRowBlock), 0, st, c.nown, c.ld, c.foff,
                                       c.adj_ptr, c.adj_low, c.adj_col, c.adj_slot, W.R, W.R2, W.D, W.G[0], W.G[1],
                                       W.ls[0], W.ly[0], W.ls[1], W.ly[1], W.uvt2, P.Craw, P.slot_ptr, P.slot_con,
                                       P.slot_a, reinterpret_cast<const double2 *>(P.slot1), W.rec, P.loc_ptr,
                                       P.loc_con, P.loc_w, reinterpret_cast<const double2 *>(P.loc1), P.b, W.cvs,
                                       W.par, ctrl_cur, inA, nA, sh ? totB : W.partB, P.mg > 0 ? (sh ? 1 : gg) : 0,
                                       ls_cur, L, W.partC, off, c.row0, P.m, pstr, k == 0 ? a.hmirror : nullptr, a.seq,
                                       P.ndense ? W.CR : nullptr, W.CD);
                else if (bfused(pb[k], tbt[k])) LRS_LAUNCH_B(LRS_BW_UB, 0);
                else LRS_LAUNCH_B(1, 1);
            });
        }
        LRS_CHECK_LAUNCH();
        off += grid;
    }
    glo = 0;
    for (int k = 0; k < KL && (mask & 4) && lat; ++k) {
        const DevCone &c = cone_of(k);
        if (lg[k].nf > 0) {
            hipLaunchKernelGGL(k_lat_f, dim3(lg[k].nf), dim3(kRowBlock), 0, st, c.ld, c.G * c.E, c.foff, c.adj_ptr,
                               c.drb, ((lg[k].nt - 64) / c.G) * kSliceB, W.gl + glo, W.D, W.G[0], W.G[1], W.ls[0], W.ly[0],
                               W.ls[1], W.ly[1], ctrl_cur, ls_cur, L, W.partC, off, P.ndense ? W.CR : nullptr, W.CD);
            LRS_CHECK_LAUNCH();
        }
        glo += (long)lg[k].sb * c.ld;
        off += lg[k].nf;
    }
    off = 0;
    for (int k = 0; k < KL && (mask & 4); ++k) {
        const DevCone &c = cone_of(k);
        const int grid = pb[k].grid;
        if (pb[k].small || bfused(pb[k], tbt[k])) { off += grid; continue; }
        if (tbt[k]) {
            static int rcb = 0;
            const int nwb = std::min(grid, resident_blocks(k_tile_b1, &rcb, kRowBlock));
            hipLaunchKernelGGL(k_tile_b1, dim3(grid), dim3(kRowBlock), 0, st, c.n, c.r, c.ld, c.foff, c.sa_items,
                               reinterpret_cast<const int4 *>(c.sa_item), c.sa_pq, c.sa_slot, W.R, W.R2, W.uvt2,
                               c.sa_S - c.slot_off, P.Craw, P.slot_ptr,
                               P.slot_con, P.slot_a,
                               reinterpret_cast<const double2 *>(P.slot1), W.rec, P.loc_ptr, P.loc_con, P.loc_w,
                               reinterpret_cast<const double2 *>(P.loc1), P.b, W.cvs, W.par, ctrl_cur, ls_cur,
                               W.partC, off, nwb);
            LRS_CHECK_LAUNCH();
            if (c.sx_n > 0) {
                hipLaunchKernelGGL(k_slot_sv, dim3(std::min(grid_elems(c.sx_n, 1), 2048)), dim3(kBlock), 0, st, c.sx_n,
                                   c.sx_slot, 0, c.sa_S - c.slot_off, P.Craw,
                                   P.slot_ptr, P.slot_con, P.slot_a,
                                   reinterpret_cast<const double2 *>(P.slot1), W.rec, W.par, ctrl_cur, ls_cur, nullptr, 0);
                LRS_CHECK_LAUNCH();
            }
            hipLaunchKernelGGL(k_tile_b2, dim3(c.sb_blocks * ((c.ld + kTbC - 1) / kTbC)), dim3(kRowBlock), 0, st, c.n, c.ld, c.foff,
                               reinterpret_cast<const int2 *>(c.sb_blk), reinterpret_cast<const int2 *>(c.sb_tp),
                               c.sb_rp, reinterpret_cast<const int2 *>(c.sb_ent), c.sa_S - c.slot_off, W.R, W.R2,
                               W.GP, P.NRpad, c.r, ctrl_cur, ls_cur, c.sb_I0);
            LRS_CHECK_LAUNCH();
            LRS_LAYOUT_SWITCH(c.G, c.E, {
                hipLaunchKernelGGL((k_wide_bf<GG, EE>), dim3(grid), dim3(kRowBlock), 0, st, c.nown, c.ld, c.foff, W.D,
                                   W.G[0], W.G[1], W.ls[0], W.ly[0], W.ls[1], W.ly[1], ctrl_cur, ls_cur, L, W.partC,
                                   offBF, c.row0, P.ndense ? W.CR : nullptr, W.CD, W.GP, P.NRpad);
            });
            offBF += grid;
        } else if (pb[k].wide) {
            LRS_LAYOUT_SWITCH(c.G, c.E, {
                if (tlb[k]) {
                    LRS_WIDE_B(true);
                    LRS_CHECK_LAUNCH();
                    hipLaunchKernelGGL((k_wide_bf<GG, EE>), dim3(grid), dim3(kRowBlock), 0, st, c.nown, c.ld, c.foff,
                                       W.D, W.G[0], W.G[1], W.ls[0], W.ly[0], W.ls[1], W.ly[1], ctrl_cur, ls_cur, L,
                                       W.partC, offBF, c.row0, P.ndense ? W.CR : nullptr, W.CD, W.GP, P.NRpad);
                    offBF += grid;
                } else {
                    LRS_WIDE_B(false);
                }
            });
        } else {
            LRS_LAYOUT_SWITCH(c.G, c.E, { LRS_LAUNCH_B(kBwU, 2); });
        }
        LRS_CHECK_LAUNCH();
// ... 1742 lines not shown
```

ltr-lowrank-sdp_amd/csrc/lrs_problem.cpp:

```cpp
#include "lrs_problem.h"

#include <hip/hip_runtime.h>

#include <algorithm>
#include <cmath>
#include <cstdio>
#include <cstdlib>
#include <cstring>
#include <fstream>
#include <sstream>

namespace lrs {

namespace {

struct RawEntry {
    int cone, con, row, col;
    double v;
};

bool is_sep(char c) {
    return c == '{' || c == '}' || c == '(' || c == ')' || c == ',' || c == '\'' || c == ' ' || c == '\t' ||
           c == '\r' || c == '\n';
}
// ... 1020 lines not shown
            std::vector<unsigned> pq(Zk);
            long t0 = 0;
            const bool swz = tile_swizzle_on();
            std::vector<long> perm;
            for (long t = 0; t < Zk; ++t) {
                pq[t] = (unsigned)(key[t].first & 0xffffffffu);
                pos[t] = key[t].second;
                const bool last = t + 1 == Zk || (key[t + 1].first >> 32) != (key[t].first >> 32) ||
                                  t + 1 - t0 == kAuvItem;
                if (!last) continue;
                const unsigned long long tile = key[t].first >> 32;
                item.push_back((int)(tile / nt) * kAuvT);
                item.push_back((int)(tile % nt) * kAuvT);
                item.push_back((int)t0);
                item.push_back((int)(t + 1));
                if (swz) {
                    swizzle_item(pq.data() + t0, t + 1 - t0, perm);
                    std::vector<unsigned> pq2(perm.size());
                    std::vector<int> pos2(perm.size());
                    for (size_t i = 0; i < perm.size(); ++i) { pq2[i] = pq[t0 + perm[i]]; pos2[i] = pos[t0 + perm[i]]; }
                    std::copy(pq2.begin(), pq2.end(), pq.begin() + t0);
                    std::copy(pos2.begin(), pos2.end(), pos.begin() + t0);
                }
                t0 = t + 1;
            }
            DevCone &d = dp.cones[k];
            d.auv_items = (int)(item.size() / 4);
            d.auv_ebase = eb;
            if (!dput(&d.auv_item, item, err) || !dput(&d.auv_pq, pq, err) || !dput(&d.auv_pos, pos, err))
                return false;
            if (hipMalloc((void **)&d.auv_val, (size_t)Zk * sizeof(double)) != hipSuccess) {
                err = "hipMalloc failed";
                return false;
            }
            if (hp.cones[k].own1 < 0) {
                const HostCone &hc = hp.cones[k];
                std::vector<int> co;
                for (size_t t = 0; t < hc.prow.size(); ++t)
                    if (hc.Chas[t]) co.push_back(d.slot_off + (int)t);
                d.cobj_n = (int)co.size();
                if (!dput(&d.cobj_slot, co, err)) return false;
            }
        }
    }
    std::vector<int> nent(m, 0), only_slot(m, -1);
    std::vector<double> only_w(m, 0.0);
    for (int k = 0; k < hp.K; ++k)
        for (int i = 0; i < m; ++i)
            for (int e = con_ptr[(long)k * m + i]; e < con_ptr[(long)k * m + i + 1]; ++e) {
                nent[i]++;
                only_slot[i] = con_slot[e];
                only_w[i] = con_w[e];
            }
    std::vector<int> glob, loc_ptr(Ptot + 1, 0), loc_con;
    std::vector<double> loc_w;
    auto is_loc = [&](int i) { return nent[i] == 1 && (hp.force_glob.empty() || !hp.force_glob[i]); };
    for (int i = 0; i < m; ++i) {
        if (is_loc(i)) loc_ptr[only_slot[i] + 1]++;
        else glob.push_back(i);
    }
    for (int t = 0; t < Ptot; ++t) loc_ptr[t + 1] += loc_ptr[t];
    loc_con.assign(loc_ptr[Ptot], 0);
    loc_w.assign(loc_ptr[Ptot], 0.0);
    {
        std::vector<int> fpl(loc_ptr.begin(), loc_ptr.end() - 1);
        for (int i = 0; i < m; ++i)
            if (is_loc(i)) {
                const int t = fpl[only_slot[i]]++;
                loc_con[t] = i;
                loc_w[t] = only_w[i];
            }
    }
    {
        std::vector<double> s1(2L * std::max(1, Ptot), 0.0), l1(2L * std::max(1, Ptot), 0.0);
        for (int t = 0; t < Ptot; ++t) {
            const int ns = slot_ptr[t + 1] - slot_ptr[t];
            s1[2L * t] = ns == 1 ? slot_a[slot_ptr[t]] : 0.0;
            s1[2L * t + 1] = ns == 0 ? -1.0 : (ns == 1 ? (double)slot_con[slot_ptr[t]] : -2.0);
            const int nl = loc_ptr[t + 1] - loc_ptr[t];
            l1[2L * t] = nl == 1 ? loc_w[loc_ptr[t]] : 0.0;
            l1[2L * t + 1] = nl == 0 ? -1.0 : (nl == 1 ? (double)loc_con[loc_ptr[t]] : -2.0);
        }
        if (!dput(&dp.slot1, s1, err) || !dput(&dp.loc1, l1, err)) return false;
    }
    dp.mg = (int)glob.size();
    dp.glob_maxlen = 0;
    for (int i : glob) dp.glob_maxlen = std::max(dp.glob_maxlen, nent[i]);
    if (glob.empty()) glob.push_back(0);
    if (loc_con.empty()) { loc_con.push_back(0); loc_w.push_back(0.0); }
    if (!dput(&dp.glob, glob, err) || !dput(&dp.loc_ptr, loc_ptr, err) || !dput(&dp.loc_con, loc_con, err) ||
        !dput(&dp.loc_w, loc_w, err))
        return false;
    if (!dput(&dp.b, hp.b, err) || !dput(&dp.Cw, Cw, err) || !dput(&dp.Craw, Craw, err) ||
        !dput(&dp.con_ptr, con_ptr, err) || !dput(&dp.con_slot, con_slot, err) || !dput(&dp.con_w, con_w, err) ||
        !dput(&dp.slot_ptr, slot_ptr, err) || !dput(&dp.slot_con, slot_con, err) || !dput(&dp.slot_a, slot_a, err))
        return false;
    if (hp.K > 1) {
        DevCone &mc = dp.merged;
        long ntot = 0, nadj = 0, Ptot_l = 0;
        for (auto &c : hp.cones) { ntot += c.n; nadj += (long)c.adj_col.size(); Ptot_l += (long)c.prow.size(); }
        std::vector<int> ap(ntot + 1, 0), al(ntot, 0), ac(nadj, 0), as(nadj, 0);
        long r0 = 0, e0 = 0;
        for (int k = 0; k < hp.K; ++k) {
            const HostCone &c = hp.cones[k];
            for (int i = 0; i < c.n; ++i) {
                ap[r0 + i] = (int)(e0 + c.adj_ptr[i]);
                al[r0 + i] = (int)(e0 + c.adj_low[i]);
            }
            for (size_t t = 0; t < c.adj_col.size(); ++t) {
                ac[e0 + t] = (int)(r0 + c.adj_col[t]);
                as[e0 + t] = dp.cones[k].slot_off + c.adj_slot[t];
            }
            r0 += c.n;
            e0 += (long)c.adj_col.size();
        }
        ap[ntot] = (int)e0;
        mc.n = (int)ntot;
        mc.nown = (int)ntot;
        mc.P = (int)Ptot_l;
        mc.adj_nnz = nadj;
        for (long q = 0; q < ntot; ++q) {
            mc.maxdeg = std::max(mc.maxdeg, ap[q + 1] - ap[q]);
            mc.maxlow = std::max(mc.maxlow, al[q] - ap[q]);
            if (al[q] - ap[q] > kDenseRow) { mc.dra_h.push_back((int)q); mc.dra_n.push_back(al[q] - ap[q]); }
            if (ap[q + 1] - ap[q] > kDenseRow) {
                mc.drb_h.push_back((int)q);
                mc.drb_n.push_back(ap[q + 1] - ap[q]);
                mc.gl_need += (long)((ap[q + 1] - ap[q] + kSliceMinB - 1) / kSliceMinB) * 256;
            }
        }
        if (!dput(&mc.dra, mc.dra_h, err) || !dput(&mc.drb, mc.drb_h, err)) return false;
        if (!dput(&mc.adj_ptr, ap, err) || !dput(&mc.adj_low, al, err) || !dput(&mc.adj_col, ac, err) ||
            !dput(&mc.adj_slot, as, err))
            return false;
        dp.has_merged = true;
    }
    for (int k = 0; k < hp.K; ++k) {
        const HostCone &c = hp.cones[k];
        DevCone &d = dp.cones[k];
        d.n = c.n;
        d.nown = c.n;
        std::vector<int> adj_slot_g(c.adj_slot.size());
        for (size_t t = 0; t < c.adj_slot.size(); ++t) adj_slot_g[t] = d.slot_off + c.adj_slot[t];
        d.adj_nnz = (long)c.adj_col.size();
        for (int q = 0; q < c.n; ++q) {
            d.maxdeg = std::max(d.maxdeg, c.adj_ptr[q + 1] - c.adj_ptr[q]);
            d.maxlow = std::max(d.maxlow, c.adj_low[q] - c.adj_ptr[q]);
            if (c.adj_low[q] - c.adj_ptr[q] > kDenseRow) {
                d.dra_h.push_back(q);
                d.dra_n.push_back(c.adj_low[q] - c.adj_ptr[q]);
            }
            if (c.adj_ptr[q + 1] - c.adj_ptr[q] > kDenseRow) {
                d.drb_h.push_back(q);
                d.drb_n.push_back(c.adj_ptr[q + 1] - c.adj_ptr[q]);
                d.gl_need += (long)((c.adj_ptr[q + 1] - c.adj_ptr[q] + kSliceMinB - 1) / kSliceMinB) * 256;
            }
        }
        if (!dput(&d.dra, d.dra_h, err) || !dput(&d.drb, d.drb_h, err)) return false;
        if (!dput(&d.adj_ptr, c.adj_ptr, err) || !dput(&d.adj_low, c.adj_low, err) ||
            !dput(&d.adj_col, c.adj_col, err) || !dput(&d.adj_slot, adj_slot_g, err))
            return false;
        if (c.own1 < 0 && c.n <= kScMaxN && (!c.dense_c || c.const_c) && !c.dense_a && !c.r1_path &&
            !upload_small_cg(c, hp.m, d, err))
            return false;
        if (c.n >= kNX && (long)c.adj_col.size() >= (long)kTileMinDeg * c.n) {
            std::vector<int> cs((size_t)c.n * (kNX + 1));
// ... 184 lines not shown
```

ltr-lowrank-sdp_amd/csrc/lrs_solver.cpp:

```cpp
#include <hip/hip_runtime.h>

#include <algorithm>
#include <atomic>
#include <chrono>
#include <cmath>
#include <cstdarg>
#include <cstdio>
#include <cstdlib>
#include <cstring>
#include <condition_variable>
#include <limits>
#include <map>
#include <mutex>
#include <string>
#include <thread>
#include <vector>

#include <rccl/rccl.h>

#include "../../include/lrsdp.h"
#include "lrs_device.h"
#include "lrs_problem.h"

namespace lrs {
// ... 2474 lines not shown
        LRS_NEED_CTX(c);                                                                  \
        if (!(c)->loaded) { set_err("%s: no problem loaded", __func__); return -1; }      \
    } while (0)
#define LRS_NEED_STATE(c)                                                                         \
    do {                                                                                          \
        LRS_NEED_LOADED(c);                                                                       \
        if (!(c)->walloc) { set_err("%s: no solver state (ranks not set)", __func__); return -1; } \
    } while (0)
#define LRS_NEED_ARG(x)                                                          \
    do {                                                                         \
        if (!(x)) { set_err("%s: null argument %s", __func__, #x); return -1; }  \
    } while (0)

void lrs_params_default(lrs_params *p) {
    if (!p) return;
    memset(p, 0, sizeof(*p));
    p->initRho = 0.0; p->rhoMax = 5000.0; p->rhoCellingALM = 1e8; p->rhoCellingADMM = 5000.0 * 200;
    p->maxALMIter = 200; p->maxADMMIter = 10000; p->timesLogRank = 2.0; p->fixedRank = -1; p->initRank = -1;
    p->rhoFreq = 5; p->rhoFactor = 1.2; p->ALMRhoFactor = 2.0; p->rankUpdateFactor = 1.5; p->phase1Tol = 1e-3;
    p->phase2Tol = 1e-5; p->timeSecLimit = 3600.0; p->heuristicFactor = 1.0; p->lbfgsListLength = 2;
    p->endTauTol = 1e-16; p->endALMSubTol = 1e-10; p->l2Rescaling = 0; p->reoptLevel = 2; p->dyrankLevel = 2;
    p->highAccMode = 0; p->oracleRankNaive = 0; p->disableOracle = 0; p->nearStallFactor = 0.0;
    p->rankSchedule = nullptr; p->rankScheduleLen = 0; p->verbose = 0; p->almInnerBudget = 0; p->skipADMM = 0;
}

const char *lrs_last_error(void) { return g_lrs_err.c_str(); }
const char *lrs_version(void) { return "lrsdp-mi355x 0.5 (abi " LRS_STR(LRSDP_ABI_VERSION) ", gfx950)"; }
int lrs_abi_version(void) { return LRSDP_ABI_VERSION; }

int lrs_ctx_create(int device, lrs_ctx **out) {
    LRS_NEED_ARG(out);
    *out = nullptr;
    lrs_ctx *c = new lrs_ctx();
    c->device = device;
    if (hipSetDevice(device) != hipSuccess) { set_err("hipSetDevice(%d) failed", device); delete c; return -1; }
    if (hipStreamCreateWithFlags(&c->st, hipStreamNonBlocking) != hipSuccess) { set_err("stream create failed"); delete c; return -1; }
    if (const char *ug = getenv("LRS_GRAPHS")) c->use_graphs = (atoi(ug) != 0);
    if (const char *sv = getenv("LRS_STATS")) c->stats = (atoi(sv) != 0);
    if (const char *cs = getenv("LRS_CG_SLACK")) c->cg_slack = std::max(0, std::min(8, atoi(cs)));
    if (const char *pb = getenv("LRS_PIPE_BATCH")) c->pipe_batch = std::max(2, std::min(64, (atoi(pb) + 1) & ~1));
    if (hipHostMalloc((void **)&c->hpin, kHpinN * sizeof(double), 0) != hipSuccess) { set_err("pinned alloc failed"); delete c; return -1; }
    if (hipMalloc((void **)&c->s_tickets, 64 * sizeof(unsigned)) != hipSuccess ||
        hipMemset(c->s_tickets, 0, 64 * sizeof(unsigned)) != hipSuccess ||
        hipMalloc((void **)&c->s_tmpfin, TF_N * sizeof(double)) != hipSuccess ||
        hipMalloc((void **)&c->s_rpart, kMaxPartialBlocks * sizeof(double)) != hipSuccess ||
        hipMalloc((void **)&c->s_fin, kFinN * sizeof(double)) != hipSuccess ||
        hipMemset(c->s_fin, 0, kFinN * sizeof(double)) != hipSuccess) {
        set_err("scratch alloc failed");
        lrs_ctx_destroy(c);
        return -1;
    }
    bind(c);
    *out = c;
    return 0;
}

int lrs_set_kernel_path(lrs_ctx *c, int path) {
    LRS_NEED_LOADED(c);
    if (path < 0 || path > 4) {
        set_err("kernel path %d: expected 0 (auto), 1 (general), 2 (general, bandwidth regime), 3 (+ long-row kernels) "
                "or 4 (the single-workgroup inner loop where it fits)", path);
        return -1;
    }
    if (c->dp.no_lat != path) {
        drop_graphs(c);
        c->dp.no_lat = path;
    }
    return 0;
}

int lrs_op_dual_infeasibility(lrs_ctx *c, double *l1, double *lam_min) {
    LRS_NEED_STATE(c);
    LRS_NEED_ARG(l1);
    return dual_infeasibility(c, l1, lam_min);
}

int lrs_get_kernel_path(lrs_ctx *c, int *used) {
    LRS_NEED_CTX(c);
    LRS_NEED_ARG(used);
    *used = c->loaded ? c->dp.last_path : -1;
    return 0;
}

int lrs_set_log_path(lrs_ctx *c, const char *path) {
    LRS_NEED_CTX(c);
    LRS_NEED_ARG(path);
    if (c->logfp) fclose(c->logfp);
    c->logfp = fopen(path, "w");
    if (!c->logfp) { set_err("cannot open log %s", path); return -1; }
    return 0;
}

void lrs_ctx_destroy(lrs_ctx *c) {
    if (!c) return;
    if (c->logfp) fclose(c->logfp);
    free_work(c);
    if (c->loaded) free_problem(c->dp);
    if (c->hpin) (void)hipHostFree(c->hpin);
    if (c->hgram) (void)hipHostFree(c->hgram);
    if (c->hmir) (void)hipHostFree(c->hmir);
    for (auto &e : c->bev)
        if (e) (void)hipEventDestroy(e);
    delete c->comm;
    for (void *q : {(void *)c->s_tickets, (void *)c->s_tmpfin, (void *)c->s_rpart, (void *)c->s_fin, (void *)c->d_sendbuf,
                    (void *)c->d_sendvec, (void *)c->Cw0, (void *)c->Craw0, (void *)c->xwg_snap})
        if (q) (void)hipFree(q);
    for (int *q : c->d_send_rows)
        if (q) (void)hipFree(q);
    bind_scratch(nullptr, nullptr, nullptr, nullptr);
    if (c->st) (void)hipStreamDestroy(c->st);
    delete c;
}

int lrs_load_sdpa(lrs_ctx *c, const char *path, double *read_seconds) {
    LRS_NEED_CTX(c);
    LRS_NEED_ARG(path);
    const double t0 = now_s();
    std::string err;
    HostProblem hp;
    if (!read_sdpa(path, hp, err)) { set_err("read_sdpa: %s", err.c_str()); return -1; }
    if (read_seconds) *read_seconds = now_s() - t0;
    free_work(c);
    if (c->loaded) free_problem(c->dp);
    c->hp = std::move(hp);
    if (!upload_problem(c->hp, c->dp, err)) { set_err("upload: %s", err.c_str()); return -1; }
    c->loaded = true;
    c->path = path;
    c->cgIterCone.assign(c->hp.K, 0);
    return 0;
}

int lrs_load_coo(lrs_ctx *c, int m, int nblk, const int *dims, const double *b, long nnz, const int *con,
                 const int *blk, const int *row, const int *col, const double *val) {
    LRS_NEED_CTX(c);
    LRS_NEED_ARG(dims);
    if (m > 0) LRS_NEED_ARG(b);
    if (nnz > 0 && (!con || !blk || !row || !col || !val)) { set_err("lrs_load_coo: null entry array"); return -1; }
    std::string err;
    HostProblem hp;
    if (!build_problem_coo(m, nblk, dims, b, nnz, con, blk, row, col, val, hp, err)) {
        set_err("load_coo: %s", err.c_str());
        return -1;
    }
    free_work(c);
    if (c->loaded) free_problem(c->dp);
    c->hp = std::move(hp);
    if (!upload_problem(c->hp, c->dp, err)) { set_err("upload: %s", err.c_str()); return -1; }
    c->loaded = true;
    c->path = "<memory>";
    c->cgIterCone.assign(c->hp.K, 0);
    return 0;
}

int lrs_load_coo_rank1(lrs_ctx *c, int m, int nblk, const int *dims, const double *b, long nnz, const int *con,
                       const int *blk, const int *row, const int *col, const double *val, int nterm, const int *tcon,
                       const int *tblk, const double *tsigma, const double *tvec) {
    LRS_NEED_CTX(c);
    LRS_NEED_ARG(dims);
    if (m > 0) LRS_NEED_ARG(b);
    if (nnz > 0 && (!con || !blk || !row || !col || !val)) { set_err("lrs_load_coo_rank1: null entry array"); return -1; }
    if (nterm > 0 && (!tcon || !tblk || !tsigma || !tvec)) { set_err("lrs_load_coo_rank1: null term array"); return -1; }
    std::string err;
    HostProblem hp;
    if (!build_problem_coo_rank1(m, nblk, dims, b, nnz, con, blk, row, col, val, nterm, tcon, tblk, tsigma, tvec, hp,
                                 err)) {
        set_err("load_coo_rank1: %s", err.c_str());
// ... 1107 lines not shown
```

ltr-lowrank-sdp_amd/solver.py:

```python
from __future__ import annotations

import ctypes as C
import json
import os
import subprocess
from pathlib import Path

import numpy as np

_HERE = Path(__file__).resolve().parent
LIB_PATH = _HERE / "_build" / "liblrsdp.so"
BIN_PATH = _HERE / "_build" / "LoRADS_v_2_0_1-alpha"

R, D, G, U, V, S0, Y0, S1, Y1 = range(9)
LAMBDA, CVS, Q1, Q2, B = range(5)


class Params(C.Structure):
    _fields_ = [
        ("initRho", C.c_double), ("rhoMax", C.c_double), ("rhoCellingALM", C.c_double),
        ("rhoCellingADMM", C.c_double), ("maxALMIter", C.c_int), ("maxADMMIter", C.c_int),
        ("timesLogRank", C.c_double), ("fixedRank", C.c_int), ("initRank", C.c_int), ("rhoFreq", C.c_int),
        ("rhoFactor", C.c_double), ("ALMRhoFactor", C.c_double), ("rankUpdateFactor", C.c_double),
        ("phase1Tol", C.c_double), ("phase2Tol", C.c_double), ("timeSecLimit", C.c_double),
# ... 2 lines not shown
        ("dyrankLevel", C.c_int), ("highAccMode", C.c_int), ("oracleRankNaive", C.c_int),
        ("disableOracle", C.c_int), ("nearStallFactor", C.c_double), ("rankSchedule", C.POINTER(C.c_int)),
        ("rankScheduleLen", C.c_int), ("verbose", C.c_int), ("almInnerBudget", C.c_long), ("skipADMM", C.c_int),
    ]


class Result(C.Structure):
    _fields_ = [
        ("alm_inner", C.c_long), ("alm_outer", C.c_long), ("admm_iter", C.c_long), ("cg_iter", C.c_long),
        ("alm_pobj", C.c_double), ("alm_dobj", C.c_double), ("alm_pinf", C.c_double), ("alm_gap", C.c_double),
        ("alm_rho", C.c_double), ("pobj", C.c_double), ("dobj", C.c_double), ("pinf", C.c_double),
        ("pinf_inf", C.c_double), ("gap", C.c_double), ("rho", C.c_double), ("solve_time", C.c_double),
        ("alm_time", C.c_double), ("admm_time", C.c_double), ("read_time", C.c_double), ("status", C.c_int),
        ("retcode", C.c_int), ("final_rank", C.c_int), ("oracle_rank", C.c_int), ("traj1_len", C.c_int),
        ("traj2_len", C.c_int), ("rho_max", C.c_double), ("dinf", C.c_double), ("dinf_inf", C.c_double),
        ("dinf_2", C.c_double), ("dinf_converged", C.c_int), ("dinf_iters", C.c_int), ("dinf_steps", C.c_long),
        ("dinf_time", C.c_double), ("obj_scale", C.c_double),
    ]

    def as_dict(self):
        return {k: getattr(self, k) for k, _ in self._fields_}


_lib = None
_HOOK = C.CFUNCTYPE(C.c_long, C.c_void_p, C.c_long)


def load_library(path=None):
    global _lib
    if _lib is not None:
        return _lib
    p = Path(path) if path else LIB_PATH
    if not p.exists():
        raise RuntimeError(f"HIP library not built: {p} (run __graft_entry__.build())")
    lib = C.CDLL(str(p))
    dp = C.POINTER(C.c_double)
    ip = C.POINTER(C.c_int)
    vp = C.c_void_p
    sig = {
        "lrs_params_default": (None, [C.POINTER(Params)]),
        "lrs_last_error": (C.c_char_p, []),
        "lrs_version": (C.c_char_p, []),
        "lrs_ctx_create": (C.c_int, [C.c_int, C.POINTER(vp)]),
        "lrs_ctx_destroy": (None, [vp]),
        "lrs_load_sdpa": (C.c_int, [vp, C.c_char_p, dp]),
        "lrs_problem_info": (C.c_int, [vp, ip, ip, ip, C.POINTER(C.c_long), C.POINTER(C.c_long)]),
        "lrs_determine_rank": (C.c_int, [vp, C.POINTER(Params), ip]),
        "lrs_set_rank": (C.c_int, [vp, ip]),
        "lrs_get_rank": (C.c_int, [vp, ip]),
        "lrs_factor_set": (C.c_int, [vp, C.c_int, dp]),
        "lrs_factor_get": (C.c_int, [vp, C.c_int, dp]),
        "lrs_vec_set": (C.c_int, [vp, C.c_int, dp]),
        "lrs_vec_get": (C.c_int, [vp, C.c_int, dp]),
        "lrs_op_q12": (C.c_int, [vp, dp, dp, dp, dp]),
        "lrs_op_constr_rr": (C.c_int, [vp, dp, dp, dp]),
        "lrs_op_grad": (C.c_int, [vp, C.c_double, dp]),
        "lrs_op_line_search": (C.c_int, [vp, C.c_double, dp, ip]),
        "lrs_op_lbfgs": (C.c_int, [vp, C.c_int, C.c_double, C.c_double]),
        "lrs_op_admm_constr": (C.c_int, [vp]),
        "lrs_op_admm_half": (C.c_int, [vp, C.c_int, C.c_int, C.c_double, C.c_double, C.c_int, ip, dp]),
        "lrs_op_dual_update": (C.c_int, [vp, C.c_double]),
        "lrs_op_gram": (C.c_int, [vp, C.c_int, C.c_int, dp]),
        "lrs_op_alm_update": (C.c_int, [vp, C.c_double, C.c_double, dp, dp]),
        "lrs_op_adjoint": (C.c_int, [vp, dp, C.c_int, dp, C.c_double, C.c_int]),
        "lrs_op_auv": (C.c_int, [vp, C.c_int, C.c_int, dp, dp]),
        "lrs_op_dimacs": (C.c_int, [vp, C.c_int, dp]),
        "lrs_abi_version": (C.c_int, []),
        "lrs_solve": (C.c_int, [vp, C.POINTER(Params), C.POINTER(Result)]),
        "lrs_trajectory": (C.c_int, [vp, C.c_int, ip, ip, C.c_int]),
        "lrs_write_json": (C.c_int, [vp, C.c_char_p, C.c_char_p, C.c_char_p, C.POINTER(Result),
                                     C.POINTER(Params)]),
        "lrs_alm_throughput": (C.c_int, [vp, C.POINTER(Params), C.c_long, C.c_long, dp, C.POINTER(C.c_long),
                                         dp, dp]),
        "lrs_set_log_path": (C.c_int, [vp, C.c_char_p]),
        "lrs_set_budget_hook": (C.c_int, [vp, _HOOK, vp]),
        "lrs_sync": (C.c_int, [vp]),
        "lrs_alm_last_step": (C.c_int, [vp, dp, ip]),
        "lrs_time_auut": (C.c_int, [vp, C.c_int, dp]),
        "lrs_profile_stages": (C.c_int, [vp, C.POINTER(Params), C.c_long, dp, C.POINTER(C.c_long)]),
        "lrs_time_stages": (C.c_int, [vp, C.c_int, dp]),
        "lrs_set_kernel_path": (C.c_int, [vp, C.c_int]),
        "lrs_op_dual_infeasibility": (C.c_int, [vp, dp, dp]),
        "lrs_get_kernel_path": (C.c_int, [vp, ip]),
        "lrs_stage_bytes": (C.c_int, [vp, dp]),
        "lrs_tile_info": (C.c_int, [vp, ip, ip]),
        "lrs_tile_used": (C.c_int, [vp, ip]),
        "lrs_auut_bytes": (C.c_int, [vp, dp]),
        "lrs_time_gram": (C.c_int, [vp, C.c_int, C.c_int, dp, dp]),
        "lrs_mfma_f64_peak": (C.c_int, [vp, dp]),
        "lrs_mfma_f64_probe": (C.c_int, [vp, C.c_int, C.c_int, dp, dp, dp]),
        "lrs_time_dense": (C.c_int, [vp, C.c_int, C.c_int, dp]),
        "lrs_dense_a_info": (C.c_int, [vp, C.c_int, ip, ip, C.POINTER(C.c_long)]),
        "lrs_time_dense_a": (C.c_int, [vp, C.c_int, C.c_int, dp]),
        "lrs_dense_a_plan": (C.c_int, [C.c_char_p, C.c_int, ip, ip, ip, C.c_int]),
        "lrs_rank1_info": (C.c_int, [vp, C.c_int, ip, ip, C.POINTER(C.c_long)]),
        "lrs_rank1_plan": (C.c_int, [C.c_char_p, C.c_int, ip, ip, ip, dp, C.c_int]),
        "lrs_time_rank1": (C.c_int, [vp, C.c_int, C.c_int, dp, dp]),
        "lrs_load_coo": (C.c_int, [vp, C.c_int, C.c_int, ip, dp, C.c_long, ip, ip, ip, ip, dp]),
        "lrs_load_coo_rank1": (C.c_int, [vp, C.c_int, C.c_int, ip, dp, C.c_long, ip, ip, ip, ip, dp, C.c_int, ip, ip,
                                         dp, dp]),
        "lrs_debug_phase_times": (C.c_int, [vp, C.POINTER(C.c_ulonglong), C.POINTER(C.c_ulonglong)]),
        "lrs_comm_unique_id": (C.c_int, [C.c_char_p]),
        "lrs_shard_rccl": (C.c_int, [vp, C.c_int, C.c_int, C.c_char_p]),
        "lrs_loopback_create": (C.c_int, [C.c_int, C.POINTER(vp)]),
        "lrs_loopback_destroy": (None, [vp]),
        "lrs_shard_loopback": (C.c_int, [vp, vp, C.c_int]),
        "lrs_shard_info": (C.c_int, [vp, ip, ip, ip, ip, ip]),
        "lrs_shard_comm_ranks": (C.c_int, [vp, ip]),
        "lrs_shard_comm_record": (C.c_int, [vp, C.c_int]),
        "lrs_xwg_fallbacks": (C.c_int, [vp, ip]),
        "lrs_shard_comm_log": (C.c_int, [vp, C.POINTER(C.c_long), C.c_long, C.POINTER(C.c_long)]),
        "lrs_shard_plan": (C.c_int, [C.c_char_p, C.c_int, C.c_int, C.POINTER(C.c_long), ip, ip, ip, ip, ip, ip, ip]),
    }
    for name, (res, args) in sig.items():
        try:
            fn = getattr(lib, name)
        except AttributeError:
            if os.environ.get("LRS_LIB"):
                continue
            raise
        fn.restype = res
        fn.argtypes = args
    _lib = lib
    return lib


def default_params(**kw):
    lib = load_library()
    p = Params()
    lib.lrs_params_default(C.byref(p))
    sched = kw.pop("rankSchedule", None)
    for k, v in kw.items():
        if not hasattr(p, k):
            raise AttributeError(k)
        setattr(p, k, v)
    if sched:
        arr = (C.c_int * len(sched))(*sched)
        p.rankSchedule = arr
        p.rankScheduleLen = len(sched)
        p._sched_keepalive = arr
    return p


def _dptr(a):
    return a.ctypes.data_as(C.POINTER(C.c_double))


def comm_unique_id():
    lib = load_library()
    buf = C.create_string_buffer(128)
    if lib.lrs_comm_unique_id(buf) != 0:
        raise RuntimeError(f"comm_unique_id: {lib.lrs_last_error().decode()}")
    return buf.raw


class LoopbackGroup:

    def __init__(self, world):
        self.lib = load_library()
        self.h = C.c_void_p()
        if self.lib.lrs_loopback_create(world, C.byref(self.h)) != 0:
            raise RuntimeError(f"loopback_create: {self.lib.lrs_last_error().decode()}")
        self.world = world

    def close(self):
        if self.h:
# ... 248 lines not shown
            st["i1"] = inner
            if on_stop:
                on_stop()
            return 0

        cb = _HOOK(hook)
        self._check(self.lib.lrs_set_budget_hook(self.ctx, cb, None), "set_budget_hook")
        try:
            res = Result()
            self._check(self.lib.lrs_solve(self.ctx, C.byref(p), C.byref(res)), "solve")
        finally:
            self.lib.lrs_set_budget_hook(self.ctx, _HOOK(), None)
        if st["t0"] is None or st["t1"] is None:
            raise RuntimeError("alm_timed: the phase-1 budget was not reached")
        return {"done": st["i1"] - st["i0"], "seconds": st["t1"] - st["t0"], "inner": res.alm_inner}

    def alm_steps(self, K, **kw):
        kw = dict(kw)
        p = default_params(**kw)
        p.maxALMIter = 1000000000
        p.skipADMM = 1
        p.timeSecLimit = 1e30
        p.almInnerBudget = int(K)
        res = Result()
        self._check(self.lib.lrs_solve(self.ctx, C.byref(p), C.byref(res)), "solve")
        out = (C.c_double * 4)()
        nw = C.c_int()
        self._check(self.lib.lrs_alm_last_step(self.ctx, out, C.byref(nw)), "alm_last_step")
        self.ranks = self.get_rank()
        pair = (S0, Y0) if nw.value == 0 else (S1, Y1)
        return {"inner": res.alm_inner, "tau": out[0], "lag": out[1], "pinf": out[2], "beta": out[3],
                "R": self.get_factor(R), "G": self.get_factor(G), "cvs": self.get_vec(CVS),
                "lam": self.get_vec(LAMBDA), "s": self.get_factor(pair[0]), "y": self.get_factor(pair[1])}

    def get_rank(self):
        out = (C.c_int * self.K)()
        self._check(self.lib.lrs_get_rank(self.ctx, out), "get_rank")
        return list(out)

    def sync(self):
        self._check(self.lib.lrs_sync(self.ctx), "sync")

    def profile_stages(self, steps, **kw):
        p = default_params(**kw)
        ms = (C.c_double * 4)()
        done = C.c_long()
        self._check(self.lib.lrs_profile_stages(self.ctx, C.byref(p), steps, ms, C.byref(done)), "profile_stages")
        return list(ms), done.value

    def auut_bytes(self):
        v = C.c_double()
        self._check(self.lib.lrs_auut_bytes(self.ctx, C.byref(v)), "auut_bytes")
        return v.value

    def tile_info(self):
        a, b = C.c_int(), C.c_int()
        self._check(self.lib.lrs_tile_info(self.ctx, C.byref(a), C.byref(b)), "tile_info")
        return a.value, b.value

    def tile_used(self):
        v = C.c_int()
        self._check(self.lib.lrs_tile_used(self.ctx, C.byref(v)), "tile_used")
        return bool(v.value)

    def stage_bytes(self):
        v = (C.c_double * 3)()
        self._check(self.lib.lrs_stage_bytes(self.ctx, v), "stage_bytes")
        return list(v)

    def set_kernel_path(self, path):
        self._check(self.lib.lrs_set_kernel_path(self.ctx, int(path)), "set_kernel_path")

    def dual_infeasibility(self):
        l1 = C.c_double()
        lm = np.zeros(max(1, len(self.dims)))
        self._check(self.lib.lrs_op_dual_infeasibility(self.ctx, C.byref(l1), _dptr(lm)), "dual_infeasibility")
        return l1.value, lm[:len(self.dims)]

    def kernel_path(self):
        v = C.c_int(-1)
        self._check(self.lib.lrs_get_kernel_path(self.ctx, C.byref(v)), "get_kernel_path")
        return v.value

    def time_stages(self, reps=200):
        ms = (C.c_double * 3)()
        self._check(self.lib.lrs_time_stages(self.ctx, reps, ms), "time_stages")
        return list(ms)

    def debug_phase_times(self):
        out = (C.c_ulonglong * 64)()
        blk = (C.c_ulonglong * (4 * 1024 * 2))()
        rc = self.lib.lrs_debug_phase_times(self.ctx, out, blk)
        if rc < 0:
            raise RuntimeError(self.lib.lrs_last_error().decode())
        if rc != 64:
            return None
        ph = [list(out[16 * k:16 * k + 16]) for k in range(4)]
        b = [[(blk[(k * 1024 + i) * 2], blk[(k * 1024 + i) * 2 + 1]) for i in range(1024)] for k in range(4)]
        return ph, b

    def time_gram(self, cone=0, reps=20):
        ms, kms = C.c_double(), C.c_double()
        self._check(self.lib.lrs_time_gram(self.ctx, cone, reps, C.byref(ms), C.byref(kms)), "time_gram")
        return ms.value, kms.value

    def time_dense(self, cone=0, reps=10):
        t = C.c_double()
        self._check(self.lib.lrs_time_dense(self.ctx, cone, reps, C.byref(t)), "time_dense")
        return t.value

    def dense_a_info(self, cone=0):
        n, on, nb = C.c_int(), C.c_int(), C.c_long()
        self._check(self.lib.lrs_dense_a_info(self.ctx, cone, C.byref(n), C.byref(on), C.byref(nb)), "dense_a_info")
        return n.value, bool(on.value), nb.value

    def time_dense_a(self, cone=0, reps=10):
        t = C.c_double()
        self._check(self.lib.lrs_time_dense_a(self.ctx, cone, reps, C.byref(t)), "time_dense_a")
        return t.value

    def rank1_info(self, cone=0):
        n, on, nb = C.c_int(), C.c_int(), C.c_long()
        self._check(self.lib.lrs_rank1_info(self.ctx, cone, C.byref(n), C.byref(on), C.byref(nb)), "rank1_info")
        return n.value, bool(on.value), nb.value

    def time_rank1(self, cone=0, reps=10):
        t, b = C.c_double(), C.c_double()
        self._check(self.lib.lrs_time_rank1(self.ctx, cone, reps, C.byref(t), C.byref(b)), "time_rank1")
        return t.value, b.value

    def mfma_f64_peak(self):
        t = C.c_double()
        self._check(self.lib.lrs_mfma_f64_peak(self.ctx, C.byref(t)), "mfma_f64_peak")
        return t.value

    def mfma_f64_probe(self, waves_per_simd=4, chains=8):
        t, f, cy = C.c_double(), C.c_double(), C.c_double()
        self._check(self.lib.lrs_mfma_f64_probe(self.ctx, int(waves_per_simd), int(chains), C.byref(t), C.byref(f),
                                                C.byref(cy)), "mfma_f64_probe")
        return t.value, f.value, cy.value

    def time_auut(self, reps=100):
        ms = C.c_double()
        self._check(self.lib.lrs_time_auut(self.ctx, reps, C.byref(ms)), "time_auut")
        return ms.value


def dense_a_plan(path, cone=0):
    lib = load_library()
    n, on = C.c_int(), C.c_int()
    if lib.lrs_dense_a_plan(str(path).encode(), cone, C.byref(n), C.byref(on), None, 0) != 0:
        raise RuntimeError(lib.lrs_last_error().decode())
    cons = np.zeros(max(1, n.value), dtype=np.int32)
    if lib.lrs_dense_a_plan(str(path).encode(), cone, C.byref(n), C.byref(on),
                            cons.ctypes.data_as(C.POINTER(C.c_int)), n.value) != 0:
        raise RuntimeError(lib.lrs_last_error().decode())
    return cons[:n.value].tolist(), bool(on.value)


def rank1_plan(path, cone=0):
    lib = load_library()
    n, on = C.c_int(), C.c_int()
    if lib.lrs_rank1_plan(str(path).encode(), cone, C.byref(n), C.byref(on), None, None, 0) != 0:
        raise RuntimeError(lib.lrs_last_error().decode())
    cons = np.zeros(max(1, n.value), dtype=np.int32)
    sig = np.zeros(max(1, n.value), dtype=np.float64)
# ... 62 lines not shown
```

Baseline: 47630 ALM inner iterations/s.

## Add specialised PLAIN variants of lattice kernels for single-constraint-per-slot problems

Adds a compile-time PLAIN template variant of k_lat_a and k_lat_b. It is selected when every slot maps to at most one constraint and no slicing, dense rows or fold paths are needed. The variant drops the slice and dense-row branches and the generic multi-constraint handling, stores per-slot results directly, and keeps base pointers and control flags in scalar registers using address-space-1 pointers and asm register hints. The goal is less branching and address arithmetic in the hot lattice kernels, at the cost of more template instantiations, added code complexity and possible changes in register pressure and occupancy.

```diff
diff --git a/include/lrsdp.h b/include/lrsdp.h
--- a/include/lrsdp.h
+++ b/include/lrsdp.h
@@ -100,6 +100,7 @@
 
 int lrs_set_kernel_path(lrs_ctx *ctx, int path);
 int lrs_get_kernel_path(lrs_ctx *ctx, int *used);
+int lrs_lat_plain_used(lrs_ctx *ctx, int *used);
 
 int lrs_time_auut(lrs_ctx *ctx, int reps, double *avg_ms);
 int lrs_auut_bytes(lrs_ctx *ctx, double *bytes);
diff --git a/ltr-lowrank-sdp_amd/csrc/lrs_device.h b/ltr-lowrank-sdp_amd/csrc/lrs_device.h
--- a/ltr-lowrank-sdp_amd/csrc/lrs_device.h
+++ b/ltr-lowrank-sdp_amd/csrc/lrs_device.h
@@ -74,6 +74,7 @@
     int row0 = 0, nown = 0;
     long foff = 0;
     int slot_off = 0, P = 0;
+    bool plain = false;
     int *adj_ptr = nullptr, *adj_low = nullptr, *adj_col = nullptr, *adj_slot = nullptr;
     long adj_nnz = 0;
     bool auv_diag = false;
@@ -154,6 +155,7 @@
     int *slot_g = nullptr;
     mutable int last_path = -1;
     mutable int last_tiles = 0;
+    mutable int last_plain = 0;
     int m = 0, K = 0;
     int lp_cone = -1;
     long NRpad = 0;
diff --git a/ltr-lowrank-sdp_amd/csrc/lrs_kernels.hip b/ltr-lowrank-sdp_amd/csrc/lrs_kernels.hip
--- a/ltr-lowrank-sdp_amd/csrc/lrs_kernels.hip
+++ b/ltr-lowrank-sdp_amd/csrc/lrs_kernels.hip
@@ -99,6 +99,23 @@
     asm volatile("" : "+v"(x));
     return x;
 }
+template <typename T>
+__device__ __forceinline__ T held(T x) {
+    asm volatile("" : "+v"(x));
+    return x;
+}
+template <typename T>
+__device__ __forceinline__ T held_s(T x) {
+    asm volatile("" : "+s"(x));
+    return x;
+}
+typedef __attribute__((address_space(1))) double gdouble;
+typedef double vdouble2 __attribute__((ext_vector_type(2)));
+typedef __attribute__((address_space(1))) vdouble2 gdouble2;
+__device__ __forceinline__ gdouble *held_gs(double *p) {
+    asm volatile("" : "+s"(p));
+    return (gdouble *)p;
+}
 
 template <int G>
 __device__ __forceinline__ double group_sum(double v) {
@@ -177,6 +194,19 @@
     } else if constexpr (E == 4) {
         reinterpret_cast<double2 *>(p)[0] = make_double2(v[0], v[1]);
         reinterpret_cast<double2 *>(p)[1] = make_double2(v[2], v[3]);
+    } else {
+#pragma unroll
+        for (int e = 0; e < E; ++e) p[e] = v[e];
+    }
+}
+
+template <int E>
+__device__ __forceinline__ void st_row(gdouble *__restrict__ p, const double (&v)[E]) {
+    if constexpr (E == 2) {
+        *reinterpret_cast<gdouble2 *>(p) = vdouble2{v[0], v[1]};
+    } else if constexpr (E == 4) {
+        reinterpret_cast<gdouble2 *>(p)[0] = vdouble2{v[0], v[1]};
+        reinterpret_cast<gdouble2 *>(p)[1] = vdouble2{v[2], v[3]};
     } else {
 #pragma unroll
         for (int e = 0; e < E; ++e) p[e] = v[e];
@@ -1159,24 +1189,32 @@
     }
 }
 
-template <int NV>
-__device__ __forceinline__ void write_partials_nw(double (&acc)[NV], double *__restrict__ part, int slot, int nw) {
+template <int NV, typename P>
+__device__ __forceinline__ P write_partials_dst(P part, int slot, int tid = threadIdx.x) {
+    return part + (long)min(tid, NV - 1) * kMaxPartialBlocks + slot;
+}
+template <int NV, typename P>
+__device__ __forceinline__ void write_partials_nw_to(double (&acc)[NV], P dst, int nw, int tid = threadIdx.x) {
     __shared__ double sh[NV][8];
-    const int wid = threadIdx.x >> 6, lane = threadIdx.x & 63;
+    const int wid = tid >> 6, lane = tid & 63;
 #pragma unroll
     for (int v = 0; v < NV; ++v) {
         const double t = wave_sum(acc[v]);
         if (lane == 0) sh[v][wid] = t;
     }
     __syncthreads();
-    if (threadIdx.x < NV) {
-        const int v = threadIdx.x;
+    if (tid < NV) {
+        const int v = tid;
         double t = 0.0;
 #pragma unroll
         for (int w = 0; w < 8; ++w)
             if (w < nw) t += sh[v][w];
-        part[v * kMaxPartialBlocks + slot] = t;
-    }
+        *dst = t;
+    }
+}
+template <int NV>
+__device__ __forceinline__ void write_partials_nw(double (&acc)[NV], double *__restrict__ part, int slot, int nw) {
+    write_partials_nw_to<NV>(acc, write_partials_dst<NV>(part, slot), nw);
 }
 
 template <int NV, int NT = kBlock>
@@ -2341,7 +2379,7 @@
     sum_partials<NV>(x, nblk, out);
 }
 
-template <int G, int E, int NO>
+template <int G, int E, int NO, bool PLAIN = false>
 __global__ void __launch_bounds__(kLatNT) k_lat_a(
     int n, int ld, long foff, const int *__restrict__ adj_ptr, const int *__restrict__ adj_low,
     const int *__restrict__ adj_col, const int *__restrict__ adj_slot, const double *__restrict__ Cw,
@@ -2363,7 +2401,7 @@
     const int nwv = lrw + 1, rpb = lrw * 64 / G;
     const bool ctrl_wave = __builtin_amdgcn_readfirstlane((int)(threadIdx.x >> 6)) == nwv - 1;
     const int lane = threadIdx.x & (G - 1);
-    const bool slice = (int)blockIdx.x >= nrb;
+    const bool slice = !PLAIN && (int)blockIdx.x >= nrb;
     int i = lat_row_block((int)blockIdx.x, nrb) * rpb + (int)threadIdx.x / G, sq = 0;
     if (slice) {
         const int per = rpb * kSliceA;
@@ -2453,7 +2491,7 @@
         ld_row<E>(R + oi, xi);
         int eb = kb, nl = valid ? ke - kb : 0;
         if (slice) { eb = kb + sq; nl = valid ? max(0, min(kSliceA, ke - eb)) : 0; }
-        else if (nl > kDenseRow) nl = 0;
+        else if (!PLAIN && nl > kDenseRow) nl = 0;
         const int kd = nl > 0 ? eb + nl - 1 : 0;
         const int jd = adj_col[kd];
         sd = adj_slot[kd];
@@ -2498,13 +2536,36 @@
             g_phase_tmp[0][2] = wall_clock64();
 #endif
     }
+    gdouble *pD = nullptr, *pRD = nullptr, *pDD = nullptr, *pRec = nullptr, *pPart = nullptr, *pCt = nullptr;
+    int wct = 0, nwh = nwv, fmg = 0, fgl = 0;
+    if constexpr (PLAIN) {
+        pD = held_gs((double *)D);
+        pRD = held_gs((double *)uRD);
+        pDD = held_gs((double *)uDD);
+        pRec = held_gs((double *)rec);
+        pPart = held_gs((double *)partA + (pblk_off + (int)blockIdx.x));
+        pCt = held_gs((double *)ctrl_cur);
+        wct = held_s(pblk_off | (int)blockIdx.x);
+        nwh = held_s(nwv);
+        fmg = held_s(__builtin_amdgcn_readfirstlane((fold && mg > 0) ? 1 : 0));
+        fgl = held_s(__builtin_amdgcn_readfirstlane((fold && do_glob && mg > 0) ? 1 : 0));
+    }
     __syncthreads();
     LRS_TS(0, 3);
-    if (pblk_off == 0 && blockIdx.x == 0 && threadIdx.x < C_NCTRL) ctrl_cur[threadIdx.x] = c[threadIdx.x];
+    if constexpr (!PLAIN) {
+        if (pblk_off == 0 && blockIdx.x == 0 && threadIdx.x < C_NCTRL) ctrl_cur[threadIdx.x] = c[threadIdx.x];
+    }
     const bool active = c[C_ACTIVE] != 0.0;
-    if (!active && !(fold && mg > 0)) return;
+    if constexpr (PLAIN) {
+        if (!active && !fmg) {
+            if (wct == 0 && threadIdx.x < C_NCTRL) pCt[threadIdx.x] = c[threadIdx.x];
+            return;
+        }
+    } else {
+        if (!active && !(fold && mg > 0)) return;
+    }
     double acc[8] = {0, 0, 0, 0, 0, 0, 0, 0};
-    if (fold && do_glob) {
+    if (PLAIN ? fgl != 0 : (fold && do_glob)) {
         if (gwide) {
             const int lane64 = threadIdx.x & 63;
             const int nw = gridDim.x * nwv;
@@ -2539,7 +2600,95 @@
             }
         }
     }
-    if (active && valid) {
+    if constexpr (PLAIN) {
+        if (active && valid) {
+            const int lane = held((int)threadIdx.x) & (G - 1);
+            DirCoef kc;
+            kc.cg = c[C_CG]; kc.cs0 = c[C_CS0]; kc.cy0 = c[C_CY0]; kc.cs1 = c[C_CS1]; kc.cy1 = c[C_CY1];
+            kc.u0 = (kc.cs0 != 0.0 || kc.cy0 != 0.0);
+            kc.u1 = (kc.cs1 != 0.0 || kc.cy1 != 0.0);
+            const double rho = pl[P_RHO], rhoInv = 1.0 / rho;
+            double yi[E];
+            own.eval(kc, yi);
+            auto pentry = [&](int j, const double (&xjv)[E], const double (&yj)[E], double cwv, double2 l1v, double bv,
+                              double cv, double lv, double &d0o, double &d1o) {
+                double d0 = 0.0, d1 = 0.0;
+                if (j != i) {
+#pragma unroll
+                    for (int e = 0; e < E; ++e) d0 += xi[e] * yj[e] + xjv[e] * yi[e];
+                    d0 *= 0.5;
+                } else {
+#pragma unroll
+                    for (int e = 0; e < E; ++e) d0 += xi[e] * yi[e];
+                }
+#pragma unroll
+                for (int e = 0; e < E; ++e) d1 += yi[e] * yj[e];
+                d0 = group_sum<G>(d0);
+                d1 = group_sum<G>(d1);
+                d0o = d0;
+                d1o = d1;
+                if (lane != 0) return;
+                acc[0] += cwv * d0;
+                acc[1] += cwv * d1;
+                const int c1 = (int)l1v.y;
+                if (c1 < 0) return;
+                const double w = l1v.x;
+                const double q1 = 2.0 * (w * d0), q2 = w * d1;
+                const double q0 = (bv - cv) + rhoInv * lv;
+                acc[2] += q2 * q2; acc[3] += q1 * q2; acc[4] += q0 * q2; acc[5] += q1 * q1;
+                acc[6] += q0 * q1;
+            };
+            auto pstore = [&](int sl, double2 l1v, double bv, double cv, double lv, double d0, double d1) {
+                pRD[sl] = d0;
+                pDD[sl] = d1;
+                const int c1 = (int)l1v.y;
+                if (c1 >= 0) {
+                    const double w = l1v.x;
+                    const double q1 = 2.0 * (w * d0), q2 = w * d1;
+                    gdouble2 *r = reinterpret_cast<gdouble2 *>(pRec + 4L * c1);
+                    r[0] = vdouble2{cv, q1};
+                    r[1] = vdouble2{q2, (-lv) + (-rho) * bv};
+                }
+            };
+            double d0v[NO + 1], d1v[NO + 1];
+#pragma unroll
+            for (int u = 0; u <= NO; ++u) d0v[u] = d1v[u] = 0.0;
+#pragma unroll
+            for (int u = 0; u < NO; ++u) {
+                if (u < no) {
+                    double yj[E];
+                    nbr[u].eval(kc, yj);
+                    pentry(jj[u], xj[u], yj, cw[u], l1[u], bq[u], cq[u], lq[u], d0v[u], d1v[u]);
+                }
+            }
+            for (int k0 = no > NO ? adj_ptr[held(ic)] : 0, k = k0 + NO; k < k0 + no; ++k) {
+                const int j = adj_col[k], sl = adj_slot[k];
+                const long oj = (long)j * ld + lane * E;
+                double xjv[E], yj[E];
+                ld_row<E>(R + oj, xjv);
+                DirRow<E> dj;
+                dj.load(kc, Gc, s0, y0, s1, y1, oj);
+                dj.eval(kc, yj);
+                const double2 l1v = loc1[sl];
+                const int ci = (int)l1v.y;
+                double bv = 0.0, cv = 0.0, lv = 0.0;
+                if (ci >= 0) { bv = b[ci]; cv = cvs[ci]; lv = lam[ci]; }
+                double d0t = 0.0, d1t = 0.0;
+                pentry(j, xjv, yj, Cw[sl], l1v, bv, cv, lv, d0t, d1t);
+                if (lane == 0) pstore(sl, l1v, bv, cv, lv, d0t, d1t);
+            }
+            if (dg) pentry(i, xi, yi, cwd, l1d, bd, cd, lmd, d0v[NO], d1v[NO]);
+            st_row<E>(pD + oi, yi);
+            if (lane == 0) {
+#pragma unroll
+                for (int u = 0; u < NO; ++u) {
+                    if (u < no) pstore(ss[u], l1[u], bq[u], cq[u], lq[u], d0v[u], d1v[u]);
+                }
+                if (dg) pstore(sd, l1d, bd, cd, lmd, d0v[NO], d1v[NO]);
+            }
+        }
+        if (wct == 0 && threadIdx.x < C_NCTRL) pCt[threadIdx.x] = c[threadIdx.x];
+    } else if (active && valid) {
         DirCoef kc;
         kc.cg = c[C_CG]; kc.cs0 = c[C_CS0]; kc.cy0 = c[C_CY0]; kc.cs1 = c[C_CS1]; kc.cy1 = c[C_CY1];
         kc.u0 = (kc.cs0 != 0.0 || kc.cy0 != 0.0);
@@ -2608,7 +2757,11 @@
         if (dg) entry(i, sd, xi, yi, cwd, l1d, bd, cd, lmd);
     }
     LRS_TS(0, 5);
-    write_partials_nw<8>(acc, partA, pblk_off + blockIdx.x, nwv);
+    if constexpr (PLAIN) {
+        const int tid = held((int)threadIdx.x);
+        write_partials_nw_to<8>(acc, write_partials_dst<8>(pPart, 0, tid), nwh, tid);
+    }
+    else write_partials_nw<8>(acc, partA, pblk_off + blockIdx.x, nwv);
     LRS_TS_END(0, 6);
 #ifdef LRS_PHASE_TIMING
     if (blockIdx.x == 0 && threadIdx.x == 0)
@@ -2617,7 +2770,7 @@
     LRS_BLK_END(0);
 }
 
-template <int G, int E, int NO>
+template <int G, int E, int NO, bool PLAIN = false>
 __global__ void __launch_bounds__(kLatNT) k_lat_b(
     int n, int ld, long foff, const int *__restrict__ adj_ptr, const int *__restrict__ adj_low,
     const int *__restrict__ adj_col, const int *__restrict__ adj_slot, double *Rb0, double *Rb1,
@@ -2641,7 +2794,7 @@
     const int nwv = lrw + 1, rpb = lrw * 64 / G;
     const bool ctrl_wave = __builtin_amdgcn_readfirstlane((int)(threadIdx.x >> 6)) == nwv - 1;
     const int lane = threadIdx.x & (G - 1);
-    const bool slice = (int)blockIdx.x >= nrb;
+    const bool slice = !PLAIN && (int)blockIdx.x >= nrb;
     int i = lat_row_block((int)blockIdx.x, nrb) * rpb + (int)threadIdx.x / G, sq = 0;
     if (slice) {
         const int per = rpb * kSliceB;
@@ -2724,7 +2877,7 @@
         if (two) { ld_row<E>(so + oi, sov); ld_row<E>(yo + oi, yov); }
         int eb = kb, nt = valid ? ke - kb : 0;
         if (slice) { eb = kb + sq; nt = valid ? max(0, min(kSliceB, ke - eb)) : 0; }
-        else if (nt > kDenseRow) { nt = 0; dense = true; }
+        else if (!PLAIN && nt > kDenseRow) { nt = 0; dense = true; }
         const int kd = (!slice && nt > 0 && kl > kb) ? kl - 1 : 0;
         const int jd = adj_col[kd];
         sd = adj_slot[kd];
@@ -2779,16 +2932,151 @@
             g_phase_tmp[2][6] = wall_clock64();
 #endif
     }
+    gdouble *pRn = nullptr, *pGn = nullptr, *pSh = nullptr, *pYh = nullptr, *pU = nullptr, *pCv = nullptr;
+    gdouble *pPart = nullptr, *pLs = nullptr;
+    int wls = 0, nwh = nwv;
+    if constexpr (PLAIN) {
+        pRn = held_gs((double *)Rn);
+        pGn = held_gs((double *)Gnew);
+        pSh = held_gs((double *)sh);
+        pYh = held_gs((double *)yh);
+        pU = held_gs((double *)uRR);
+        pCv = held_gs((double *)cvs);
+        pPart = held_gs((double *)partC + (pblk_off + (int)blockIdx.x));
+        pLs = held_gs((double *)ls_cur);
+        wls = held_s(pblk_off | (int)blockIdx.x);
+        nwh = held_s(nwv);
+    }
     __syncthreads();
     LRS_TS(2, 2);
-    if (pblk_off == 0 && blockIdx.x == 0 && threadIdx.x < LS_N) ls_cur[threadIdx.x] = ls[threadIdx.x];
-    if (ls[LS_FLAG] != 0.0) return;
-    const double tau = ls[LS_TAU], tau2 = tau * tau, rho = par[P_RHO];
+    if constexpr (!PLAIN) {
+        if (pblk_off == 0 && blockIdx.x == 0 && threadIdx.x < LS_N) ls_cur[threadIdx.x] = ls[threadIdx.x];
+    }
+    if (ls[LS_FLAG] != 0.0) {
+        if constexpr (PLAIN) {
+            if (wls == 0 && threadIdx.x < LS_N) pLs[threadIdx.x] = ls[threadIdx.x];
+        }
+        return;
+    }
+    const double tau = ls[LS_TAU], tau2 = tau * tau;
+    double rho;
+    if constexpr (PLAIN) rho = pl[P_RHO];
+    else rho = par[P_RHO];
     double acc[10] = {0, 0, 0, 0, 0, 0, 0, 0, 0, 0};
     double g[E];
 #pragma unroll
     for (int e = 0; e < E; ++e) g[e] = 0.0;
-    if (valid) {
+    if constexpr (PLAIN) {
+        if (valid) {
+            const int lane = held((int)threadIdx.x) & (G - 1);
+#pragma unroll
+            for (int e = 0; e < E; ++e) ri[e] += tau * di[e];
+            auto pentry = [&](bool lower, const double (&rj)[E], double svv, double2 s1u, double2 ra_, double2 rb_,
+                              double2 l1u, double bv, double &dv) {
+                if ((int)s1u.y >= 0) {
+                    double cv = ra_.x + tau * ra_.y;
+                    cv = cv + tau2 * rb_.x;
+                    const double M1 = rb_.y + rho * cv;
+                    svv += M1 * s1u.x;
+                }
+#pragma unroll
+                for (int e = 0; e < E; ++e) g[e] += svv * rj[e];
+                if (!lower) return;
+                double d = 0.0;
+#pragma unroll
+                for (int e = 0; e < E; ++e) d += ri[e] * rj[e];
+                d = group_sum<G>(d);
+                dv = d;
+                const int cl = (int)l1u.y;
+                if (lane != 0 || cl < 0) return;
+                const double tot = l1u.x * d;
+                const double dd = bv - tot;
+                acc[9] += dd * dd;
+            };
+            auto pstore = [&](int sl, double2 l1u, double d) {
+                pU[sl] = d;
+                const int cl = (int)l1u.y;
+                if (cl >= 0) pCv[cl] = l1u.x * d;
+            };
+            double dv[NO + 1];
+#pragma unroll
+            for (int u = 0; u <= NO; ++u) dv[u] = 0.0;
+#pragma unroll
+            for (int u = 0; u < NO; ++u) {
+                if (u < no) {
+                    double rj[E];
+#pragma unroll
+                    for (int e = 0; e < E; ++e) rj[e] = rjp[u][e] + tau * djp[u][e];
+                    pentry(lw[u], rj, sv[u], s1v[u], ra[u], rb[u], l1v[u], bq[u], dv[u]);
+                }
+            }
+            if (no > NO) {
+                const int ih = held(ic);
+                const int kb = adj_ptr[ih], kl = adj_low[ih], ke = adj_ptr[ih + 1];
+                int cnt = 0;
+                for (int k = kb; k < ke; ++k) {
+                    if (dg && k == kl - 1) continue;
+                    if (cnt++ < NO) continue;
+                    const int j = adj_col[k], sl = adj_slot[k];
+                    const long oj = (long)j * ld + lane * E;
+                    double rj[E], dj[E];
+                    ld_row<E>(R + oj, rj);
+                    ld_row<E>(D + oj, dj);
+#pragma unroll
+                    for (int e = 0; e < E; ++e) rj[e] += tau * dj[e];
+                    const double2 s1u = slot1[sl];
+                    const int c1 = (int)s1u.y;
+                    double2 x = make_double2(0.0, 0.0), y = x;
+                    if (c1 >= 0) {
+                        const double2 *r = reinterpret_cast<const double2 *>(rec + 4L * c1);
+                        x = r[0];
+                        y = r[1];
+                    }
+                    const bool lower = k < kl;
+                    const double2 l1u = lower ? loc1[sl] : make_double2(0.0, -1.0);
+                    const int cl = (int)l1u.y;
+                    double dt = 0.0;
+                    pentry(lower, rj, Craw[sl], s1u, x, y, l1u, cl >= 0 ? b[cl] : 0.0, dt);
+                    if (lower && lane == 0) pstore(sl, l1u, dt);
+                }
+            }
+            if (dg) pentry(true, ri, svd, s1d, rad, rbd, l1d, bqd, dv[NO]);
+            double sv2[E], yv[E];
+#pragma unroll
+            for (int e = 0; e < E; ++e) g[e] *= 2.0;
+#pragma unroll
+            for (int e = 0; e < E; ++e) { sv2[e] = tau * di[e]; yv[e] = g[e] - go[e]; }
+#pragma unroll
+            for (int e = 0; e < E; ++e) {
+                acc[0] += g[e] * g[e];
+                acc[1] += yv[e] * sv2[e];
+                acc[2] += yv[e] * yv[e];
+                acc[3] += sv2[e] * g[e];
+                acc[4] += yv[e] * g[e];
+            }
+            if (two) {
+#pragma unroll
+                for (int e = 0; e < E; ++e) {
+                    acc[5] += sov[e] * g[e];
+                    acc[6] += yov[e] * g[e];
+                    acc[7] += sov[e] * yv[e];
+                    acc[8] += yov[e] * yv[e];
+                }
+            }
+            st_row<E>(pRn + oi, ri);
+            st_row<E>(pGn + oi, g);
+            st_row<E>(pSh + oi, sv2);
+            st_row<E>(pYh + oi, yv);
+            if (lane == 0) {
+#pragma unroll
+                for (int u = 0; u < NO; ++u) {
+                    if (u < no && lw[u]) pstore(ss[u], l1v[u], dv[u]);
+                }
+                if (dg) pstore(sd, l1d, dv[NO]);
+            }
+        }
+        if (wls == 0 && threadIdx.x < LS_N) pLs[threadIdx.x] = ls[threadIdx.x];
+    } else if (valid) {
 #pragma unroll
         for (int e = 0; e < E; ++e) ri[e] += tau * di[e];
         if (!slice) st_row<E>(Rn + oi, ri);
@@ -2918,7 +3206,11 @@
         }
     }
     LRS_TS(2, 3);
-    write_partials_nw<10>(acc, partC, pblk_off + blockIdx.x, nwv);
+    if constexpr (PLAIN) {
+        const int tid = held((int)threadIdx.x);
+        write_partials_nw_to<10>(acc, write_partials_dst<10>(pPart, 0, tid), nwh, tid);
+    }
+    else write_partials_nw<10>(acc, partC, pblk_off + blockIdx.x, nwv);
     LRS_TS_END(2, 4);
 #ifdef LRS_PHASE_TIMING
     if (blockIdx.x == 0 && threadIdx.x == 0)
@@ -5415,12 +5707,16 @@
 template <int GG, int EE>
 static int res_la() {
     static int c = 0;
-    return resident_blocks(k_lat_a<GG, EE, kLatNoA>, &c, kLatNT);
+    static int cp = 0;
+    return std::min(resident_blocks(k_lat_a<GG, EE, kLatNoA>, &c, kLatNT),
+                    resident_blocks(k_lat_a<GG, EE, kLatNoA, true>, &cp, kLatNT));
 }
 template <int GG, int EE>
 static int res_lb() {
     static int c = 0;
-    return resident_blocks(k_lat_b<GG, EE, kLatNoB>, &c, kLatNT);
+    static int cp = 0;
+    return std::min(resident_blocks(k_lat_b<GG, EE, kLatNoB>, &c, kLatNT),
+                    resident_blocks(k_lat_b<GG, EE, kLatNoB, true>, &cp, kLatNT));
 }
 static bool lat_disabled() {
     static int v = -1;
@@ -5462,6 +5758,11 @@
     lp.nt = 64 * (w + 1);
     return lp;
 }
+static bool lat_plain(const DevProblem &P, const DevCone &c, const LatPlan &lp) {
+    const char *e = getenv("LRS_LAT_PLAIN");
+    if (e && e[0] == '0') return false;
+    return c.plain && lp.sa == 0 && lp.sb == 0 && lp.nf == 0 && c.dra_h.empty() && c.drb_h.empty() && !P.ndense;
+}
 static int lat_forced_waves() {
     static int forced = -1;
     if (forced < 0) {
@@ -5633,6 +5934,9 @@
         lat = false;
     P.last_path = lat ? 0 : 1;
     P.last_tiles = 0;
+    P.last_plain = lat ? 1 : 0;
+    for (int k = 0; k < KL && lat; ++k)
+        if (!lat_plain(P, cone_of(k), lg[k])) P.last_plain = 0;
     for (int k = 0; k < KL; ++k)
         if (tbt[k] || (pa[k].wide && !merge && !tla[k] && cone_of(k).sa_items > 0)) P.last_tiles = 1;
     if (lat) {
@@ -5691,15 +5995,20 @@
                        W.uvt2, W.par, ctrl_prev, ctrl_cur, ls_prev, inC, nC, W.part, off, pa[k].T, gwide, c.row0, \
                        pstr)
         if (lat) {
+#define LRS_LAT_A(PL_)                                                                                         \
+    hipLaunchKernelGGL((k_lat_a<GG, EE, kLatNoA, PL_>), dim3(grid), dim3(lg[k].nt), 0, st, c.nown, c.ld, c.foff,   \
+                       c.adj_ptr, c.adj_low, c.adj_col, c.adj_slot, P.Cw, W.R, W.R2, W.D, W.G[0], W.G[1], W.ls[0], \
+                       W.ly[0], W.ls[1], W.ly[1], W.uvt0, W.uvt1, P.loc_ptr, P.loc_con, P.loc_w,                 \
+                       reinterpret_cast<const double2 *>(P.loc1), P.b, W.cvs, W.lam, W.rec, k == 0 ? 1 : 0, P.mg,   \
+                       P.glob, P.m, P.K, P.con_ptr, P.con_slot, P.con_w, W.uvt2, W.par, ctrl_prev, ctrl_cur,       \
+                       ls_prev, inC, nC, W.part, off, gwide, lg[k].nrb, lg[k].nt / 64 - 1, (int)c.dra_h.size(),    \
+                       c.dra)
+            const bool plain = lat_plain(P, c, lg[k]);
             LRS_LAYOUT_SWITCH(c.G, c.E, {
-                hipLaunchKernelGGL((k_lat_a<GG, EE, kLatNoA>), dim3(grid), dim3(lg[k].nt), 0, st, c.nown,
-                                   c.ld, c.foff, c.adj_ptr, c.adj_low, c.adj_col, c.adj_slot, P.Cw, W.R, W.R2, W.D,
-                                   W.G[0], W.G[1], W.ls[0], W.ly[0], W.ls[1], W.ly[1], W.uvt0, W.uvt1, P.loc_ptr,
-                                   P.loc_con, P.loc_w, reinterpret_cast<const double2 *>(P.loc1), P.b, W.cvs, W.lam,
-                                   W.rec, k == 0 ? 1 : 0, P.mg, P.glob, P.m, P.K, P.con_ptr, P.con_slot, P.con_w,
-                                   W.uvt2, W.par, ctrl_prev, ctrl_cur, ls_prev, inC, nC, W.part, off, gwide,
-                                   lg[k].nrb, lg[k].nt / 64 - 1, (int)c.dra_h.size(), c.dra);
+                if (plain) LRS_LAT_A(true);
+                else LRS_LAT_A(false);
             });
+#undef LRS_LAT_A
         } else {
             LRS_LAYOUT_SWITCH(c.G, c.E, {
                 if (split) LRS_LAUNCH_A(1, 1);
@@ -5785,16 +6094,21 @@
                        (MM) != 2 && k == 0 ? a.hmirror : nullptr, a.seq, P.ndense ? W.CR : nullptr, W.CD)
         const bool small = pb[k].small;
         if (lat) {
+#define LRS_LAT_B(PL_)                                                                                         \
+    hipLaunchKernelGGL((k_lat_b<GG, EE, kLatNoB, PL_>), dim3(grid), dim3(lg[k].nt), 0, st, c.nown, c.ld, c.foff,   \
+                       c.adj_ptr, c.adj_low, c.adj_col, c.adj_slot, W.R, W.R2, W.D, W.G[0], W.G[1], W.ls[0],       \
+                       W.ly[0], W.ls[1], W.ly[1], W.uvt2, P.Craw, P.slot_ptr, P.slot_con, P.slot_a,               \
+                       reinterpret_cast<const double2 *>(P.slot1), W.rec, P.loc_ptr, P.loc_con, P.loc_w,           \
+                       reinterpret_cast<const double2 *>(P.loc1), P.b, W.cvs, W.par, ctrl_cur, inA, nA, W.partB,    \
+                       P.mg > 0 ? gg : 0, ls_cur, L, W.partC, off, P.m, k == 0 ? a.hmirror : nullptr, a.seq,        \
+                       lg[k].nrb, lg[k].nt / 64 - 1, (int)c.drb_h.size(), c.drb, W.gl + glo,                       \
+                       P.ndense ? W.CR : nullptr, W.CD)
+            const bool plain = lat_plain(P, c, lg[k]);
             LRS_LAYOUT_SWITCH(c.G, c.E, {
-                hipLaunchKernelGGL((k_lat_b<GG, EE, kLatNoB>), dim3(grid), dim3(lg[k].nt), 0, st, c.nown,
-                                   c.ld, c.foff, c.adj_ptr, c.adj_low, c.adj_col, c.adj_slot, W.R, W.R2, W.D, W.G[0],
-                                   W.G[1], W.ls[0], W.ly[0], W.ls[1], W.ly[1], W.uvt2, P.Craw, P.slot_ptr, P.slot_con,
-                                   P.slot_a, reinterpret_cast<const double2 *>(P.slot1), W.rec, P.loc_ptr, P.loc_con,
-                                   P.loc_w, reinterpret_cast<const double2 *>(P.loc1), P.b, W.cvs, W.par, ctrl_cur,
-                                   inA, nA, W.partB, P.mg > 0 ? gg : 0, ls_cur, L, W.partC, off, P.m,
-                                   k == 0 ? a.hmirror : nullptr, a.seq, lg[k].nrb, lg[k].nt / 64 - 1, (int)c.drb_h.size(), c.drb,
-                                   W.gl + glo, P.ndense ? W.CR : nullptr, W.CD);
+                if (plain) LRS_LAT_B(true);
+                else LRS_LAT_B(false);
             });
+#undef LRS_LAT_B
             glo += (long)lg[k].sb * c.ld;
         } else {
             LRS_LAYOUT_SWITCH(c.G, c.E, {
diff --git a/ltr-lowrank-sdp_amd/csrc/lrs_problem.cpp b/ltr-lowrank-sdp_amd/csrc/lrs_problem.cpp
--- a/ltr-lowrank-sdp_amd/csrc/lrs_problem.cpp
+++ b/ltr-lowrank-sdp_amd/csrc/lrs_problem.cpp
@@ -1126,6 +1126,14 @@
             l1[2L * t + 1] = nl == 0 ? -1.0 : (nl == 1 ? (double)loc_con[loc_ptr[t]] : -2.0);
         }
         if (!dput(&dp.slot1, s1, err) || !dput(&dp.loc1, l1, err)) return false;
+        dp.merged.plain = true;
+        for (int k = 0; k < hp.K; ++k) {
+            DevCone &d = dp.cones[k];
+            d.plain = true;
+            for (int t = d.slot_off; t < d.slot_off + d.P; ++t)
+                if (s1[2L * t + 1] == -2.0 || l1[2L * t + 1] == -2.0) d.plain = false;
+            if (!d.plain) dp.merged.plain = false;
+        }
     }
     dp.mg = (int)glob.size();
     dp.glob_maxlen = 0;
diff --git a/ltr-lowrank-sdp_amd/csrc/lrs_solver.cpp b/ltr-lowrank-sdp_amd/csrc/lrs_solver.cpp
--- a/ltr-lowrank-sdp_amd/csrc/lrs_solver.cpp
+++ b/ltr-lowrank-sdp_amd/csrc/lrs_solver.cpp
@@ -2580,6 +2580,13 @@
     return 0;
 }
 
+int lrs_lat_plain_used(lrs_ctx *c, int *used) {
+    LRS_NEED_CTX(c);
+    LRS_NEED_ARG(used);
+    *used = (c->loaded && c->dp.last_path == 0) ? c->dp.last_plain : 0;
+    return 0;
+}
+
 int lrs_set_log_path(lrs_ctx *c, const char *path) {
     LRS_NEED_CTX(c);
     LRS_NEED_ARG(path);
diff --git a/ltr-lowrank-sdp_amd/solver.py b/ltr-lowrank-sdp_amd/solver.py
--- a/ltr-lowrank-sdp_amd/solver.py
+++ b/ltr-lowrank-sdp_amd/solver.py
@@ -108,6 +108,7 @@
         "lrs_set_kernel_path": (C.c_int, [vp, C.c_int]),
         "lrs_op_dual_infeasibility": (C.c_int, [vp, dp, dp]),
         "lrs_get_kernel_path": (C.c_int, [vp, ip]),
+        "lrs_lat_plain_used": (C.c_int, [vp, ip]),
         "lrs_stage_bytes": (C.c_int, [vp, dp]),
         "lrs_tile_info": (C.c_int, [vp, ip, ip]),
         "lrs_tile_used": (C.c_int, [vp, ip]),
@@ -522,6 +523,11 @@
         self._check(self.lib.lrs_get_kernel_path(self.ctx, C.byref(v)), "get_kernel_path")
         return v.value
 
+    def lat_plain_used(self):
+        v = C.c_int(0)
+        self._check(self.lib.lrs_lat_plain_used(self.ctx, C.byref(v)), "lat_plain_used")
+        return bool(v.value)
+
     def time_stages(self, reps=200):
         ms = (C.c_double * 3)()
         self._check(self.lib.lrs_time_stages(self.ctx, reps, ms), "time_stages")
```

New measurement: 51820 ALM inner iterations/s, median of 6. 1.09x the previous value.
